# nasa-nccs-hpda/super-resolution-climate

Measured on NVIDIA B200. Metric: rcan_train_tiles_per_s, higher is better.
Workload: dtype bf16

## Files before the change

include/sres_b200.h:

```cpp
#ifndef SRES_B200_H_
#define SRES_B200_H_

#include <stddef.h>
#include <stdint.h>

#ifdef __cplusplus
extern "C" {
#endif

#define SRES_API __attribute__((visibility("default")))

#define SRES_OK 0
#define SRES_ERR_INVALID_ARG 1
#define SRES_ERR_UNSUPPORTED 2
#define SRES_ERR_CUDA 3
#define SRES_ERR_NO_DEVICE 4

#define SRES_NF 64

SRES_API int sres_abi_version(void);
SRES_API const char* sres_last_error(void);
SRES_API int sres_device_sm_count(void);
SRES_API long long sres_launch_count(void);
SRES_API int sres_l2_set_aside(size_t bytes);
SRES_API int sres_l2_persist_window(const void* base, size_t bytes, void* stream);
SRES_API int sres_profile_report(char* buf, size_t nbuf);
SRES_API int64_t sres_ptl_rows(int B, int H, int W);

#define SRES_EPI_RELU 1u
#define SRES_EPI_POOL 2u
#define SRES_EPI_DOT 4u

#define SRES_MAP_IDENT 0
#define SRES_MAP_SHUFFLE 1
#define SRES_MAP_UNSHUFFLE 2

typedef struct sres_conv_args {
  const void* in_bf16;
  const void* wpack_bf16;
  const float* bias;
  const float* resid_f32;
  const float* resid2_f32;
  const void* mask_bf16;
  float* out_f32;
  void* out_bf16;
  float* pool_part;
  float* out_nchw;
  int32_t B, H, W;
  int32_t n_out;
  int32_t c_real;
  uint32_t epi_flags;
  int32_t map_mode;
  int32_t sub_i, sub_j;
  int32_t shuffle_factor;
  int32_t debug_flags;
  void* debug_timeline;
} sres_conv_args;

SRES_API int sres_conv_tile_rows(int H, int W);
SRES_API int sres_conv_mtiles(int B, int H, int W);
SRES_API int sres_conv_supported(int H, int W, int n_out);
SRES_API int sres_conv3x3_igemm(const sres_conv_args* args, void* stream);

SRES_API size_t sres_conv_pair_flag_bytes(int B, int H, int W);
SRES_API int sres_conv_pair_supported(const sres_conv_args* first, const sres_conv_args* second);
SRES_API int sres_conv3x3_pair(const sres_conv_args* first, const sres_conv_args* second, void* flags, void* stream);

typedef struct sres_rcab_chain_args {
  void* xb_bf16;
  void* t1_bf16;
  void* t2_bf16;
  const void* wpack_bf16;
  const float* params;
  const float* x_in_f32;
  float* x_f32;
  float* save_mean;
  float* save_s;
  void* scratch;
  int64_t rcab_stride, save_stride;
  int32_t B, H, W, n_blocks, hidden;
  int32_t xb_first, xb_ring, xb_count;
  int32_t t_first, t_fixed, t_count;
  void* debug_timeline;
} sres_rcab_chain_args;
SRES_API int sres_rcab_chain_supported(int B, int H, int W);
SRES_API size_t sres_rcab_chain_scratch_bytes(int B);
SRES_API int sres_rcab_chain_fwd(const sres_rcab_chain_args* args, void* stream);

SRES_API int sres_pack_conv_weights(const float* w_oihw, void* out_bf16, int mode, int n_rows, int cin,
                           int cout_total, int oc_stride, int oc_offset, void* stream);

SRES_API size_t sres_conv_wgrad_workspace_bytes(void);
#define SRES_WGRAD_MAX_JOBS 8
typedef struct sres_wgrad_job {
  const void* x_bf16;
  const void* dy_bf16;
  float* dw_oihw;
  float* dbias;
  int32_t cout_total, oc_stride, oc_offset, accumulate;
  float scale;
} sres_wgrad_job;
SRES_API int sres_conv3x3_wgrad_batch(const sres_wgrad_job* jobs, int njobs, int B, int H, int W, void* workspace,
                                      size_t workspace_bytes, void* stream);
SRES_API int sres_conv3x3_wgrad(const void* x_bf16, const void* dy_bf16, int B, int H, int W, float* dw_oihw,
                                float* dbias, int cout_total, int oc_stride, int oc_offset, int accumulate,
                                void* workspace, size_t workspace_bytes, void* stream);

SRES_API int sres_conv3x3_small_in(const float* in_nchw, const float* w, const float* bias, int B, int Cs, int H,
                                   int W, int transposed, int unshuffle, float* out_f32, void* out_bf16,
                                   void* stream);
SRES_API int sres_conv3x3_small_out(const void* u_bf16, const float* w, const float* bias, int B, int Cs, int H, int W,
                                    float* out_nchw, void* stream);
SRES_API size_t sres_small_wgrad_workspace_bytes(void);
SRES_API int sres_small_in_wgrad(const float* g1_f32, const float* g2_f32, const float* in_nchw, int B, int Cs,
                                 int H, int W, float* dw, float* db, int accumulate, void* workspace,
                                 size_t workspace_bytes, void* stream);
SRES_API int sres_small_out_wgrad(const float* dout_nchw, const void* u_bf16, int B, int Cs, int H, int W,
                                  float* dw, float* db, int accumulate, void* workspace, size_t workspace_bytes,
                                  void* stream);

SRES_API int sres_ca_blocks_per_image(int B, int H, int W);
SRES_API int sres_ca_pool(const void* t2_bf16, float* pool_sum, int B, int H, int W, void* stream);
SRES_API int sres_ca_apply_fwd(const void* t2_bf16, const float* pool_part, const float* pool_sum, const float* w1,
                               const float* b1, const float* w2, const float* b2, int hidden, const float* x_in,
                               float* x_out, void* xb_out_bf16, float* save_mean, float* save_s, int B, int H, int W,
                               void* stream);
SRES_API int sres_ca_apply_fwd_split(const void* t2_bf16, const float* pool_part, const float* pool_sum, const float* w1,
                                     const float* b1, const float* w2, const float* b2, int hidden, const float* x_in_f32,
                                     const void* xhi_in_bf16, const void* xlo_in_bf16, void* xhi_out_bf16,
                                     void* xlo_out_bf16, float* save_mean, float* save_s, int B, int H, int W,
                                     void* stream);
SRES_API int sres_ca_bwd(const float* grad_f32, const void* t2_bf16, const float* w1, const float* b1,
                         const float* w2, const float* b2, int hidden, const float* save_mean, float* ds_part,
                         void* dt2_bf16, float* save_ds, int B, int H, int W, void* stream);
SRES_API int sres_ca_bwd_apply(const float* grad_f32, const float* tile_part, const float* w1, const float* b1,
                               const float* w2, const float* b2, int hidden, const float* save_mean, void* dt2_bf16,
                               float* save_ds, int B, int H, int W, void* stream);
SRES_API size_t sres_ca_param_grads_scratch_bytes(int nlayers, int B);
SRES_API int sres_ca_param_grads(const float* params_first, float* grads_first, int64_t layer_stride, int nlayers,
                                 const float* save_mean, const float* save_ds, int B, int hidden, int accumulate,
                                 void* scratch, size_t scratch_bytes, void* stream);

SRES_API int sres_bicubic_resize(const float* in, float* out, int planes, int Hi, int Wi, int Ho, int Wo,
                                 double scale_h, double scale_w, void* stream);

SRES_API size_t sres_loss_workspace_bytes(void);
SRES_API int sres_loss_sum(const float* prd, const float* tgt, int planes, int H, int W, int tH, int tW, int kind,
                           double* stat, void* workspace, size_t workspace_bytes, void* stream);
SRES_API int sres_loss_value(const double* stat, double n_total, const double* n_total_dev, int kind, float* loss,
                             void* stream);
SRES_API int sres_loss_grad(const float* prd, const float* tgt, int planes, int H, int W, int tH, int tW, int kind,
                            const float* loss, double n_total, const double* n_total_dev, float gscale,
                            const float* gscale_dev, float* grad,
                            void* stream);

SRES_API int sres_adam_step_flat(float* p, const float* g, float* m, float* v, int64_t n, int64_t step, double lr,
                                 double beta1, double beta2, double eps, double weight_decay, void* stream);

#define SRES_ARCH_RCAN 0
#define SRES_ARCH_EDSR 1
typedef struct sres_rcan_desc {
  int32_t B, H, W;
  int32_t cin, cout;
  int32_t nfeatures;
  int32_t n_groups;
  int32_t n_blocks;
  int32_t reduction;
  int32_t n_up;
  int32_t up_factor[4];
  int32_t arch;
  float res_scale;
} sres_rcan_desc;

SRES_API int64_t sres_rcan_param_count(const sres_rcan_desc* d);
SRES_API int sres_rcan_workspace_bytes(const sres_rcan_desc* d, int training, size_t* bytes);
SRES_API int sres_rcan_pack_weights(const sres_rcan_desc* d, const float* params, void* workspace, int training,
                                    void* stream);
SRES_API int sres_rcan_forward(const sres_rcan_desc* d, const float* params, const float* x_nchw, float* out_nchw,
                               void* workspace, int training, void* stream);
SRES_API int sres_rcan_num_segments(const sres_rcan_desc* d);
SRES_API int sres_rcan_segment_params(const sres_rcan_desc* d, int seg, int64_t* offset, int64_t* count);
SRES_API int sres_async_create(void** ctx);
SRES_API int sres_async_destroy(void* ctx);
SRES_API int sres_rcan_backward(const sres_rcan_desc* d, const float* params, const float* x_nchw,
                                const float* dout_nchw, float* grads, int accumulate, void* workspace, int seg_begin,
                                int seg_end, void* async_ctx, void* stream);

SRES_API int sres_tiles_finite_flags(const float* region, int C, int Y, int X, int y0, int x0, int T, int gy, int gx,
                                     int32_t* flags, void* stream);
SRES_API int sres_tiles_gather(const float* region, int C, int Y, int X, int y0, int x0, int T, int gy, int gx,
                               const int32_t* src_tile, int nslots, float* out, void* stream);
SRES_API int sres_tiles_lnorm(const float* in, int nplanes, int T, int flip_index, float* out, float* mean,
                              float* std_, void* stream);
SRES_API int sres_tiles_stitch(const float* tiles, int C, int ivar, int t, int gy, int gx, const int32_t* cell_to_tile,
                               const float* mean, const float* std_, float* out, void* stream);

SRES_API size_t sres_llc_index_workspace_bytes(int nx);
SRES_API int sres_llc_build_roi_index(const void* template_be, int nx, int y0, int ys, int x0, int xs, void* workspace,
                                      size_t workspace_bytes, int32_t* roi_index, int64_t* n_ocean_dev, void* stream);
SRES_API int sres_llc_gather_roi(const void* data_be, int64_t n_data, const int32_t* roi_index, int64_t npix, float* out,
                                 void* stream);

#ifdef __cplusplus
}
#endif
#endif
```

super-resolution-climate_b200/csrc/ca.cu:

```cuda
#include "internal.h"
#include "ptx.cuh"

namespace sres {

constexpr int kCaThreads = 256;
constexpr int kCaMaxHidden = 64;

struct CaGeom {
  int B, H, W, P, RP;
  int hid;
  int blocks_per_image;
  int tile_rows;
};

__device__ __forceinline__ float warp_sum(float v) {
#pragma unroll
  for (int o = 16; o > 0; o >>= 1) v += __shfl_xor_sync(0xffffffffu, v, o);
  return v;
}
__device__ __forceinline__ void ca_mlp(const float* __restrict__ w1, const float* __restrict__ b1,
                                       const float* __restrict__ w2, const float* __restrict__ b2, int hid,
                                       const float* sm_m, float* sm_h, float* sm_z, float* sm_s) {
  const int lane = threadIdx.x & 31, wrp = threadIdx.x >> 5;
  const float m0 = sm_m[lane], m1 = sm_m[lane + 32];
  for (int j = wrp; j < hid; j += kCaThreads / 32) {
    const float v = warp_sum(fmaf(__ldg(w1 + j * 64 + lane), m0, __ldg(w1 + j * 64 + 32 + lane) * m1));
    if (lane == 0) sm_h[j] = fmaxf(v + __ldg(b1 + j), 0.f);
  }
  __syncthreads();
  for (int c = wrp; c < 64; c += kCaThreads / 32) {
    float v = lane < hid ? __ldg(w2 + c * hid + lane) * sm_h[lane] : 0.f;
    if (lane + 32 < hid) v = fmaf(__ldg(w2 + c * hid + lane + 32), sm_h[lane + 32], v);
    v = warp_sum(v);
    if (lane == 0) {
      const float z = v + __ldg(b2 + c);
      sm_z[c] = z;
      sm_s[c] = 1.f / (1.f + expf(-z));
    }
  }
  __syncthreads();
}

struct CaWeights {
  float* w1;
  float* w2t;
  float* b1;
  float* b2;
};
static size_t ca_weights_bytes(int hid) { return (size_t)(2 * hid * 64 + hid + 64) * sizeof(float); }
__device__ __forceinline__ void ca_stage_weights(CaWeights& S, const float* __restrict__ w1, const float* __restrict__ b1,
                                                 const float* __restrict__ w2, const float* __restrict__ b2, int hid) {
  extern __shared__ float ca_dyn_smem[];
  S.w1 = ca_dyn_smem; S.w2t = S.w1 + hid * 64; S.b1 = S.w2t + hid * 64; S.b2 = S.b1 + hid;
  for (int i = threadIdx.x; i < hid * 64; i += kCaThreads) {
    S.w1[i] = __ldg(w1 + i);
    S.w2t[(i % hid) * 64 + i / hid] = __ldg(w2 + i);
  }
  if (threadIdx.x < hid) S.b1[threadIdx.x] = __ldg(b1 + threadIdx.x);
  if (threadIdx.x < 64) S.b2[threadIdx.x] = __ldg(b2 + threadIdx.x);
}
__device__ __forceinline__ void ca_hidden(const CaWeights& S, int hid, const float* sm_m, float* sm_h) {
  const int lane = threadIdx.x & 31, wrp = threadIdx.x >> 5;
  const float m0 = sm_m[lane], m1 = sm_m[lane + 32];
  for (int j = wrp; j < hid; j += kCaThreads / 32) {
    const float v = warp_sum(fmaf(S.w1[j * 64 + lane], m0, S.w1[j * 64 + 32 + lane] * m1));
    if (lane == 0) sm_h[j] = fmaxf(v + S.b1[j], 0.f);
  }
}
__device__ __forceinline__ float ca_gate(const CaWeights& S, int hid, const float* sm_h, int c) {
  float z = S.b2[c];
  for (int j = 0; j < hid; ++j) z = fmaf(S.w2t[j * 64 + c], sm_h[j], z);
  return 1.f / (1.f + expf(-z));
}

__global__ void __launch_bounds__(kCaThreads)
ca_pool_kernel(CaGeom g, const uint16_t* __restrict__ t2, float* __restrict__ pool_sum) {
  __shared__ float sm[kCaThreads / 8][64 + 1];
  const int b = blockIdx.x, tid = threadIdx.x, cg = tid & 7;
  float a[8] = {0, 0, 0, 0, 0, 0, 0, 0};
  for (int r = tid >> 3; r < g.RP; r += kCaThreads / 8) {
    const uint4 tv = *reinterpret_cast<const uint4*>(t2 + ((size_t)b * g.RP + r) * 64 + cg * 8);
    a[0] += bf16_lo(tv.x); a[1] += bf16_hi(tv.x); a[2] += bf16_lo(tv.y); a[3] += bf16_hi(tv.y);
    a[4] += bf16_lo(tv.z); a[5] += bf16_hi(tv.z); a[6] += bf16_lo(tv.w); a[7] += bf16_hi(tv.w);
  }
#pragma unroll
  for (int j = 0; j < 8; ++j) sm[tid >> 3][cg * 8 + j] = a[j];
  __syncthreads();
  if (tid < 64) {
    float s = 0.f;
    for (int i = 0; i < kCaThreads / 8; ++i) s += sm[i][tid];
    pool_sum[b * 64 + tid] = s;
  }
}


template <bool kSplit>
__global__ void __launch_bounds__(kCaThreads)
ca_apply_fwd_kernel(CaGeom g, const uint16_t* __restrict__ t2, const float* __restrict__ pool_part,
                    const float* __restrict__ pool_sum, const float* __restrict__ w1, const float* __restrict__ b1,
                    const float* __restrict__ w2, const float* __restrict__ b2, const float* x_in, float* x_out,
                    uint16_t* __restrict__ xb_out, float* __restrict__ save_mean, float* __restrict__ save_s,
                    const uint16_t* __restrict__ xhi_in, const uint16_t* xlo_in, uint16_t* xlo_out) {
  __shared__ float sm_red[4][64];
  __shared__ float sm_m[64], sm_h[kCaMaxHidden], sm_s[64];
  CaWeights sw;
  const int b = blockIdx.y, tid = threadIdx.x;
  const int cg = tid & 7;
  ca_stage_weights(sw, w1, b1, w2, b2, g.hid);
  pdl_wait();
  pdl_launch_dependents();
  const int per_blk = (g.RP + g.blocks_per_image - 1) / g.blocks_per_image;
  const int r0 = blockIdx.x * per_blk + (tid >> 3), r1 = min(g.RP, blockIdx.x * per_blk + per_blk);
  if (pool_sum) {
    sm_red[tid >> 6][tid & 63] = (tid < 64) ? pool_sum[b * 64 + tid] : 0.f;
  } else {
    const int c = tid & 63, part = tid >> 6;
    const int t0 = (b * g.RP) / g.tile_rows, t1 = ((b + 1) * g.RP - 1) / g.tile_rows;
    float a = 0.f;
#pragma unroll 8
    for (int t = t0; t <= t1; ++t) {
      const int seg = (t * g.tile_rows >= b * g.RP) ? 0 : 1;
      a += pool_part[(((size_t)t * 2 + seg) * 4 + part) * 64 + c];
    }
    sm_red[part][c] = a;
  }
  __syncthreads();
  if (tid < 64) sm_m[tid] = (sm_red[0][tid] + sm_red[1][tid] + sm_red[2][tid] + sm_red[3][tid]) / float(g.H * g.W);
  __syncthreads();
  ca_hidden(sw, g.hid, sm_m, sm_h);
  __syncthreads();
  if (tid < 64) {
    const float sg = ca_gate(sw, g.hid, sm_h, tid);
    sm_s[tid] = sg;
    if (blockIdx.x == 0) {
      save_mean[b * 64 + tid] = sm_m[tid];
      save_s[b * 64 + tid] = sg;
    }
  }
  __syncthreads();
  if constexpr (kSplit) {
    float s8[8];
#pragma unroll
    for (int j = 0; j < 8; ++j) s8[j] = sm_s[cg * 8 + j];
#pragma unroll 2
    for (int r = r0; r < r1; r += kCaThreads / 8) {
      const size_t q = (size_t)b * g.RP + r;
      const uint4 tv = *reinterpret_cast<const uint4*>(t2 + q * 64 + cg * 8);
      float x[8];
      if (x_in) {
        const float4 xa = *reinterpret_cast<const float4*>(x_in + q * 64 + cg * 8);
        const float4 xb = *reinterpret_cast<const float4*>(x_in + q * 64 + cg * 8 + 4);
        x[0] = xa.x; x[1] = xa.y; x[2] = xa.z; x[3] = xa.w; x[4] = xb.x; x[5] = xb.y; x[6] = xb.z; x[7] = xb.w;
      } else {
        const uint4 hv = *reinterpret_cast<const uint4*>(xhi_in + q * 64 + cg * 8);
        const uint4 lv = *reinterpret_cast<const uint4*>(xlo_in + q * 64 + cg * 8);
        x[0] = bf16_lo(hv.x) + bf16_lo(lv.x); x[1] = bf16_hi(hv.x) + bf16_hi(lv.x);
        x[2] = bf16_lo(hv.y) + bf16_lo(lv.y); x[3] = bf16_hi(hv.y) + bf16_hi(lv.y);
        x[4] = bf16_lo(hv.z) + bf16_lo(lv.z); x[5] = bf16_hi(hv.z) + bf16_hi(lv.z);
        x[6] = bf16_lo(hv.w) + bf16_lo(lv.w); x[7] = bf16_hi(hv.w) + bf16_hi(lv.w);
      }
      float o[8];
      o[0] = fmaf(bf16_lo(tv.x), s8[0], x[0]); o[1] = fmaf(bf16_hi(tv.x), s8[1], x[1]);
      o[2] = fmaf(bf16_lo(tv.y), s8[2], x[2]); o[3] = fmaf(bf16_hi(tv.y), s8[3], x[3]);
      o[4] = fmaf(bf16_lo(tv.z), s8[4], x[4]); o[5] = fmaf(bf16_hi(tv.z), s8[5], x[5]);
      o[6] = fmaf(bf16_lo(tv.w), s8[6], x[6]); o[7] = fmaf(bf16_hi(tv.w), s8[7], x[7]);
      const uint4 h = make_uint4(pack_bf16x2(o[0], o[1]), pack_bf16x2(o[2], o[3]), pack_bf16x2(o[4], o[5]), pack_bf16x2(o[6], o[7]));
      *reinterpret_cast<uint4*>(xb_out + q * 64 + cg * 8) = h;
      *reinterpret_cast<uint4*>(xlo_out + q * 64 + cg * 8) =
          make_uint4(pack_bf16x2(o[0] - bf16_lo(h.x), o[1] - bf16_hi(h.x)), pack_bf16x2(o[2] - bf16_lo(h.y), o[3] - bf16_hi(h.y)),
                     pack_bf16x2(o[4] - bf16_lo(h.z), o[5] - bf16_hi(h.z)), pack_bf16x2(o[6] - bf16_lo(h.w), o[7] - bf16_hi(h.w)));
    }
  } else {
  float s8[8];
#pragma unroll
  for (int j = 0; j < 4; ++j) { s8[j] = sm_s[cg * 4 + j]; s8[4 + j] = sm_s[32 + cg * 4 + j]; }
#pragma unroll 2
  for (int r = r0; r < r1; r += kCaThreads / 8) {
    const size_t q = (size_t)b * g.RP + r;
    const uint2 ta = *reinterpret_cast<const uint2*>(t2 + q * 64 + cg * 4);
    const uint2 tb = *reinterpret_cast<const uint2*>(t2 + q * 64 + 32 + cg * 4);
    const float4 xa = *reinterpret_cast<const float4*>(x_in + q * 64 + cg * 4);
    const float4 xb = *reinterpret_cast<const float4*>(x_in + q * 64 + 32 + cg * 4);
    float o[8];
    o[0] = fmaf(bf16_lo(ta.x), s8[0], xa.x); o[1] = fmaf(bf16_hi(ta.x), s8[1], xa.y);
    o[2] = fmaf(bf16_lo(ta.y), s8[2], xa.z); o[3] = fmaf(bf16_hi(ta.y), s8[3], xa.w);
    o[4] = fmaf(bf16_lo(tb.x), s8[4], xb.x); o[5] = fmaf(bf16_hi(tb.x), s8[5], xb.y);
    o[6] = fmaf(bf16_lo(tb.y), s8[6], xb.z); o[7] = fmaf(bf16_hi(tb.y), s8[7], xb.w);
    *reinterpret_cast<float4*>(x_out + q * 64 + cg * 4) = make_float4(o[0], o[1], o[2], o[3]);
    *reinterpret_cast<float4*>(x_out + q * 64 + 32 + cg * 4) = make_float4(o[4], o[5], o[6], o[7]);
    if (xb_out) {
      *reinterpret_cast<uint2*>(xb_out + q * 64 + cg * 4) = make_uint2(pack_bf16x2(o[0], o[1]), pack_bf16x2(o[2], o[3]));
      *reinterpret_cast<uint2*>(xb_out + q * 64 + 32 + cg * 4) = make_uint2(pack_bf16x2(o[4], o[5]), pack_bf16x2(o[6], o[7]));
    }
  }
  }
}

__global__ void __launch_bounds__(kCaThreads)
ca_bwd_reduce_kernel(CaGeom g, const float* __restrict__ grad, const uint16_t* __restrict__ t2,
                     float* __restrict__ ds_part) {
  __shared__ float sm[kCaThreads / 8][64 + 1];
  pdl_wait();
  pdl_launch_dependents();
  const int b = blockIdx.y, tid = threadIdx.x, cg = tid & 7;
  const int per_blk = (g.RP + g.blocks_per_image - 1) / g.blocks_per_image;
  const int r0 = blockIdx.x * per_blk, r1 = min(g.RP, r0 + per_blk);
  float a[8] = {0, 0, 0, 0, 0, 0, 0, 0};
  for (int r = r0 + (tid >> 3); r < r1; r += kCaThreads / 8) {
    const size_t q = (size_t)b * g.RP + r;
    const uint2 ta = *reinterpret_cast<const uint2*>(t2 + q * 64 + cg * 4);
    const uint2 tb = *reinterpret_cast<const uint2*>(t2 + q * 64 + 32 + cg * 4);
    const float4 ga = *reinterpret_cast<const float4*>(grad + q * 64 + cg * 4);
    const float4 gb = *reinterpret_cast<const float4*>(grad + q * 64 + 32 + cg * 4);
    a[0] = fmaf(ga.x, bf16_lo(ta.x), a[0]); a[1] = fmaf(ga.y, bf16_hi(ta.x), a[1]);
    a[2] = fmaf(ga.z, bf16_lo(ta.y), a[2]); a[3] = fmaf(ga.w, bf16_hi(ta.y), a[3]);
    a[4] = fmaf(gb.x, bf16_lo(tb.x), a[4]); a[5] = fmaf(gb.y, bf16_hi(tb.x), a[5]);
    a[6] = fmaf(gb.z, bf16_lo(tb.y), a[6]); a[7] = fmaf(gb.w, bf16_hi(tb.y), a[7]);
  }
#pragma unroll
  for (int j = 0; j < 4; ++j) { sm[tid >> 3][cg * 4 + j] = a[j]; sm[tid >> 3][32 + cg * 4 + j] = a[4 + j]; }
  __syncthreads();
  if (tid < 64) {
    float s = 0.f;
    for (int i = 0; i < kCaThreads / 8; ++i) s += sm[i][tid];
    ds_part[((size_t)b * g.blocks_per_image + blockIdx.x) * 64 + tid] = s;
  }
}

__global__ void __launch_bounds__(kCaThreads)
ca_bwd_apply_kernel(CaGeom g, const float* __restrict__ grad, const float* __restrict__ ds_part,
                    const float* __restrict__ tile_part, const float* __restrict__ w1, const float* __restrict__ b1, const float* __restrict__ w2,
                    const float* __restrict__ b2, const float* __restrict__ save_mean,
                    uint16_t* __restrict__ dt2, float* __restrict__ save_ds) {
  __shared__ float sm_m[64], sm_h[kCaMaxHidden], sm_s[64], sm_dz[64], sm_dh[kCaMaxHidden], sm_dm[64];
  __shared__ float sm_dsr[4][64];
  CaWeights sw;
  const int b = blockIdx.y, tid = threadIdx.x;
  const int lane = tid & 31, wrp = tid >> 5, cg = tid & 7;
  ca_stage_weights(sw, w1, b1, w2, b2, g.hid);
  pdl_wait();
  pdl_launch_dependents();
  const int per_blk = (g.RP + g.blocks_per_image - 1) / g.blocks_per_image;
  const int r0 = blockIdx.x * per_blk + (tid >> 3), r1 = min(g.RP, blockIdx.x * per_blk + per_blk);
  if (tile_part) {
    const int c = tid & 63, part = tid >> 6;
    const int t0 = (b * g.RP) / g.tile_rows, t1 = ((b + 1) * g.RP - 1) / g.tile_rows;
    float a = 0.f;
#pragma unroll 8
    for (int t = t0; t <= t1; ++t) {
      const int seg = (t * g.tile_rows >= b * g.RP) ? 0 : 1;
      a += tile_part[(((size_t)t * 2 + seg) * 4 + part) * 64 + c];
    }
    sm_dsr[part][c] = a;
  } else if (tid < 64) {
    float a = 0.f;
    for (int i = 0; i < g.blocks_per_image; ++i) a += ds_part[((size_t)b * g.blocks_per_image + i) * 64 + tid];
    sm_dsr[0][tid] = a;
    sm_dsr[1][tid] = sm_dsr[2][tid] = sm_dsr[3][tid] = 0.f;
  }
  if (tid < 64) sm_m[tid] = save_mean[b * 64 + tid];
  __syncthreads();
  ca_hidden(sw, g.hid, sm_m, sm_h);
  __syncthreads();
  if (tid < 64) {
    const float ds = (sm_dsr[0][tid] + sm_dsr[1][tid]) + (sm_dsr[2][tid] + sm_dsr[3][tid]);
    if (blockIdx.x == 0) save_ds[b * 64 + tid] = ds;
    const float sg = ca_gate(sw, g.hid, sm_h, tid);
    sm_s[tid] = sg;
    sm_dz[tid] = ds * sg * (1.f - sg);
  }
  __syncthreads();
  for (int j = wrp; j < g.hid; j += kCaThreads / 32) {
    const float v = warp_sum(fmaf(sw.w2t[j * 64 + lane], sm_dz[lane], sw.w2t[j * 64 + 32 + lane] * sm_dz[lane + 32]));
    if (lane == 0) sm_dh[j] = sm_h[j] > 0.f ? v : 0.f;
  }
  __syncthreads();
  if (tid < 64) {
    float a = 0.f;
    for (int j = 0; j < g.hid; ++j) a = fmaf(sw.w1[j * 64 + tid], sm_dh[j], a);
    sm_dm[tid] = a / float(g.H * g.W);
  }
  __syncthreads();
  float s8[8], m8[8];
#pragma unroll
  for (int j = 0; j < 4; ++j) {
    s8[j] = sm_s[cg * 4 + j]; s8[4 + j] = sm_s[32 + cg * 4 + j];
    m8[j] = sm_dm[cg * 4 + j]; m8[4 + j] = sm_dm[32 + cg * 4 + j];
  }
  int y = r0 / g.P, x = r0 - y * g.P;
#pragma unroll 4
  for (int r = r0; r < r1; r += kCaThreads / 8) {
    const size_t q = (size_t)b * g.RP + r;
    const float4 ga = *reinterpret_cast<const float4*>(grad + q * 64 + cg * 4);
    const float4 gb = *reinterpret_cast<const float4*>(grad + q * 64 + 32 + cg * 4);
    const bool valid = (x != g.W) && (y != g.H);
    uint2 oa, ob;
    oa.x = pack_bf16x2(fmaf(ga.x, s8[0], m8[0]), fmaf(ga.y, s8[1], m8[1]));
    oa.y = pack_bf16x2(fmaf(ga.z, s8[2], m8[2]), fmaf(ga.w, s8[3], m8[3]));
    ob.x = pack_bf16x2(fmaf(gb.x, s8[4], m8[4]), fmaf(gb.y, s8[5], m8[5]));
    ob.y = pack_bf16x2(fmaf(gb.z, s8[6], m8[6]), fmaf(gb.w, s8[7], m8[7]));
    if (!valid) { oa = make_uint2(0, 0); ob = make_uint2(0, 0); }
    *reinterpret_cast<uint2*>(dt2 + q * 64 + cg * 4) = oa;
    *reinterpret_cast<uint2*>(dt2 + q * 64 + 32 + cg * 4) = ob;
    x += kCaThreads / 8;
    while (x >= g.P) { x -= g.P; ++y; }
  }
}

struct CaParamBatch {
  const float* params;
  float* grads;
  long long layer_stride;
  const float* mean;
  const float* ds;
};

__global__ void __launch_bounds__(kCaThreads)
ca_param_prep_kernel(const CaParamBatch batch, int B, int hid, float* __restrict__ scratch) {
  __shared__ float sm_m[64], sm_h[kCaMaxHidden], sm_z[64], sm_s[64], sm_dz[64];
  const int layer = blockIdx.x, b = blockIdx.y, tid = threadIdx.x;
  const long long o = (long long)layer * batch.layer_stride;
  const float* w1 = batch.params + o;
  const float* b1 = w1 + hid * 64;
  const float* w2 = b1 + hid;
  const float* b2 = w2 + 64 * hid;
  if (tid < 64) sm_m[tid] = batch.mean[((size_t)layer * B + b) * 64 + tid];
  __syncthreads();
  ca_mlp(w1, b1, w2, b2, hid, sm_m, sm_h, sm_z, sm_s);
  float* out = scratch + ((size_t)layer * B + b) * (64 + 2 * kCaMaxHidden);
  if (tid < 64) {
    const float s = sm_s[tid];
    const float dz = batch.ds[((size_t)layer * B + b) * 64 + tid] * s * (1.f - s);
    sm_dz[tid] = dz;
    out[tid] = dz;
  }
  __syncthreads();
  if (tid < hid) {
    float a = 0.f;
    for (int c = 0; c < 64; ++c) a = fmaf(w2[c * hid + tid], sm_dz[c], a);
    out[64 + tid] = sm_h[tid];
    out[64 + kCaMaxHidden + tid] = sm_h[tid] > 0.f ? a : 0.f;
  }
}

constexpr int kCaParamChunk = 32;
__global__ void __launch_bounds__(kCaThreads)
ca_param_sum_kernel(const CaParamBatch batch, int B, int hid, const float* __restrict__ scratch, int accumulate) {
  __shared__ float sm[kCaParamChunk][4][64];
  const int layer = blockIdx.x, tid = threadIdx.x;
  const long long o = (long long)layer * batch.layer_stride;
  float* dw1 = batch.grads + o;
  float* db1 = dw1 + hid * 64;
  float* dw2 = db1 + hid;
  float* db2 = dw2 + 64 * hid;
  const int n12 = hid * 64;
  float a1[16], a2[16];
#pragma unroll
  for (int i = 0; i < 16; ++i) a1[i] = a2[i] = 0.f;
  float ab1 = 0.f, ab2 = 0.f;
  for (int b0 = 0; b0 < B; b0 += kCaParamChunk) {
    const int nb = min(kCaParamChunk, B - b0);
    __syncthreads();
    for (int i = tid; i < nb * 256; i += kCaThreads) {
      const int b = i >> 8, k = (i >> 6) & 3, c = i & 63;
      const size_t img = (size_t)layer * B + b0 + b;
      sm[b][k][c] = k < 3 ? scratch[img * (64 + 2 * kCaMaxHidden) + k * 64 + c] : batch.mean[img * 64 + c];
    }
    __syncthreads();
    for (int b = 0; b < nb; ++b) {
      const float* dz = sm[b][0];
      const float* h = sm[b][1];
      const float* dh = sm[b][2];
      const float* m = sm[b][3];
#pragma unroll
      for (int i = 0; i < 16; ++i) {
        const int e = tid + i * kCaThreads;
        if (e < n12) {
          a1[i] = fmaf(dh[e / 64], m[e % 64], a1[i]);
          a2[i] = fmaf(dz[e / hid], h[e % hid], a2[i]);
        }
      }
      if (tid < hid) ab1 += dh[tid];
      if (tid < 64) ab2 += dz[tid];
    }
  }
#pragma unroll
  for (int i = 0; i < 16; ++i) {
    const int e = tid + i * kCaThreads;
    if (e < n12) {
      dw1[e] = accumulate ? dw1[e] + a1[i] : a1[i];
      dw2[e] = accumulate ? dw2[e] + a2[i] : a2[i];
    }
  }
  if (tid < hid) db1[tid] = accumulate ? db1[tid] + ab1 : ab1;
  if (tid < 64) db2[tid] = accumulate ? db2[tid] + ab2 : ab2;
}

static int ca_geom(CaGeom* g, int B, int H, int W, int hid) {
  if (B <= 0 || H <= 0 || W <= 0) return set_error(SRES_ERR_INVALID_ARG, "ca: bad geometry");
  if (hid < 1 || hid > kCaMaxHidden) return set_error(SRES_ERR_UNSUPPORTED, "ca: hidden width must be 1..64");
  g->B = B; g->H = H; g->W = W; g->P = W + 1; g->RP = (H + 1) * (W + 1); g->hid = hid;
  int sms = device_sm_count();
  if (sms <= 0) sms = 148;
  int bpi = (4 * sms + B - 1) / B;
  const int max_bpi = (g->RP + 31) / 32;
  if (bpi > max_bpi) bpi = max_bpi;
  if (bpi < 1) bpi = 1;
  g->blocks_per_image = bpi;
  g->tile_rows = sres_conv_tile_rows(H, W);
  return SRES_OK;
}

}

using namespace sres;

extern "C" int sres_ca_blocks_per_image(int B, int H, int W) {
  CaGeom g;
  if (ca_geom(&g, B, H, W, 1)) return -1;
  return g.blocks_per_image;
}

extern "C" int sres_ca_pool(const void* t2_bf16, float* pool_sum, int B, int H, int W, void* stream) {
  CaGeom g;
  int rc = ca_geom(&g, B, H, W, 1);
  if (rc) return rc;
  if (!t2_bf16 || !pool_sum) return set_error(SRES_ERR_INVALID_ARG, "ca_pool: null pointer");
  ca_pool_kernel<<<B, kCaThreads, 0, (cudaStream_t)stream>>>(g, (const uint16_t*)t2_bf16, pool_sum);
  SRES_CHECK_LAUNCH("ca_pool: launch");
  return SRES_OK;
}

extern "C" int sres_ca_apply_fwd(const void* t2_bf16, const float* pool_part, const float* pool_sum, const float* w1, const float* b1,
                                 const float* w2, const float* b2, int hidden, const float* x_in, float* x_out,
                                 void* xb_out_bf16, float* save_mean, float* save_s, int B, int H, int W,
                                 void* stream) {
  CaGeom g;
  int rc = ca_geom(&g, B, H, W, hidden);
  if (rc) return rc;
  if (!pool_sum && g.RP < 128) return set_error(SRES_ERR_UNSUPPORTED, "ca_apply_fwd: fused pool partials need (H+1)*(W+1) >= 128; pass pool_sum");
  if (!t2_bf16 || (!pool_part && !pool_sum) || !w1 || !b1 || !w2 || !b2 || !x_in || !x_out || !save_mean || !save_s)
    return set_error(SRES_ERR_INVALID_ARG, "ca_apply_fwd: null pointer");
  dim3 grid(g.blocks_per_image, B);
  cudaError_t e = launch_pdl_if(pdl_level() >= 2, ca_apply_fwd_kernel<false>, grid, dim3(kCaThreads), ca_weights_bytes(hidden), (cudaStream_t)stream, g, (const uint16_t*)t2_bf16,
                             pool_part, pool_sum, w1, b1, w2, b2, x_in, x_out, (uint16_t*)xb_out_bf16, save_mean, save_s,
                             (const uint16_t*)nullptr, (const uint16_t*)nullptr, (uint16_t*)nullptr);
  if (e != cudaSuccess) return set_cuda_error(e, "ca_apply_fwd: launch");
  return SRES_OK;
}

extern "C" int sres_ca_apply_fwd_split(const void* t2_bf16, const float* pool_part, const float* pool_sum, const float* w1,
                                       const float* b1, const float* w2, const float* b2, int hidden, const float* x_in_f32,
                                       const void* xhi_in_bf16, const void* xlo_in_bf16, void* xhi_out_bf16,
                                       void* xlo_out_bf16, float* save_mean, float* save_s, int B, int H, int W,
                                       void* stream) {
  CaGeom g;
  int rc = ca_geom(&g, B, H, W, hidden);
  if (rc) return rc;
  if (!pool_sum && g.RP < 128) return set_error(SRES_ERR_UNSUPPORTED, "ca_apply_fwd_split: fused pool partials need (H+1)*(W+1) >= 128; pass pool_sum");
  if (!t2_bf16 || (!pool_part && !pool_sum) || !w1 || !b1 || !w2 || !b2 || !xhi_out_bf16 || !xlo_out_bf16 || !save_mean || !save_s)
    return set_error(SRES_ERR_INVALID_ARG, "ca_apply_fwd_split: null pointer");
  if ((x_in_f32 != nullptr) == (xhi_in_bf16 != nullptr || xlo_in_bf16 != nullptr) || (!x_in_f32 && (!xhi_in_bf16 || !xlo_in_bf16)))
    return set_error(SRES_ERR_INVALID_ARG, "ca_apply_fwd_split: pass either x_in_f32 or both xhi_in_bf16 and xlo_in_bf16");
  if (xhi_in_bf16 == xhi_out_bf16) return set_error(SRES_ERR_INVALID_ARG, "ca_apply_fwd_split: xhi_out must not alias xhi_in");
  dim3 grid(g.blocks_per_image, B);
  cudaError_t e = launch_pdl_if(pdl_level() >= 2, ca_apply_fwd_kernel<true>, grid, dim3(kCaThreads), ca_weights_bytes(hidden), (cudaStream_t)stream, g, (const uint16_t*)t2_bf16,
                             pool_part, pool_sum, w1, b1, w2, b2, x_in_f32, (float*)nullptr, (uint16_t*)xhi_out_bf16, save_mean, save_s,
                             (const uint16_t*)xhi_in_bf16, (const uint16_t*)xlo_in_bf16, (uint16_t*)xlo_out_bf16);
  if (e != cudaSuccess) return set_cuda_error(e, "ca_apply_fwd_split: launch");
  return SRES_OK;
}

extern "C" int sres_ca_bwd(const float* grad_f32, const void* t2_bf16, const float* w1, const float* b1,
                           const float* w2, const float* b2, int hidden, const float* save_mean, float* ds_part,
                           void* dt2_bf16, float* save_ds, int B, int H, int W, void* stream) {
  CaGeom g;
  int rc = ca_geom(&g, B, H, W, hidden);
  if (rc) return rc;
  if (!grad_f32 || !t2_bf16 || !w1 || !b1 || !w2 || !b2 || !save_mean || !ds_part || !dt2_bf16 || !save_ds)
    return set_error(SRES_ERR_INVALID_ARG, "ca_bwd: null pointer");
  dim3 grid(g.blocks_per_image, B);
  cudaError_t e = launch_pdl_if(pdl_level() >= 2, ca_bwd_reduce_kernel, grid, dim3(kCaThreads), 0, (cudaStream_t)stream, g, grad_f32,
                             (const uint16_t*)t2_bf16, ds_part);
  if (e != cudaSuccess) return set_cuda_error(e, "ca_bwd: reduce launch");
  e = launch_pdl_if(pdl_level() >= 2, ca_bwd_apply_kernel, grid, dim3(kCaThreads), ca_weights_bytes(hidden), (cudaStream_t)stream, g, grad_f32, (const float*)ds_part, (const float*)nullptr, w1, b1,
                 w2, b2, save_mean, (uint16_t*)dt2_bf16, save_ds);
  if (e != cudaSuccess) return set_cuda_error(e, "ca_bwd: apply launch");
  return SRES_OK;
}

extern "C" int sres_ca_bwd_apply(const float* grad_f32, const float* tile_part, const float* w1, const float* b1,
                                 const float* w2, const float* b2, int hidden, const float* save_mean, void* dt2_bf16,
                                 float* save_ds, int B, int H, int W, void* stream) {
  CaGeom g;
  int rc = ca_geom(&g, B, H, W, hidden);
  if (rc) return rc;
  if (g.RP < 128) return set_error(SRES_ERR_UNSUPPORTED, "ca_bwd_apply: per-tile partials need (H+1)*(W+1) >= 128");
  if (!grad_f32 || !tile_part || !w1 || !b1 || !w2 || !b2 || !save_mean || !dt2_bf16 || !save_ds)
    return set_error(SRES_ERR_INVALID_ARG, "ca_bwd_apply: null pointer");
  dim3 grid(g.blocks_per_image, B);
  cudaError_t e = launch_pdl_if(pdl_level() >= 2, ca_bwd_apply_kernel, grid, dim3(kCaThreads), ca_weights_bytes(hidden), (cudaStream_t)stream, g, grad_f32,
                                (const float*)nullptr, tile_part, w1, b1, w2, b2, save_mean, (uint16_t*)dt2_bf16, save_ds);
  if (e != cudaSuccess) return set_cuda_error(e, "ca_bwd_apply: launch");
  return SRES_OK;
}

extern "C" size_t sres_ca_param_grads_scratch_bytes(int nlayers, int B) {
  return (size_t)(nlayers > 0 ? nlayers : 0) * (B > 0 ? B : 0) * (64 + 2 * kCaMaxHidden) * sizeof(float);
}

extern "C" int sres_ca_param_grads(const float* params_first, float* grads_first, int64_t layer_stride, int nlayers,
                                   const float* save_mean, const float* save_ds, int B, int hidden, int accumulate,
                                   void* scratch, size_t scratch_bytes, void* stream) {
  if (!params_first || !grads_first || !save_mean || !save_ds || !scratch || nlayers <= 0 || B <= 0)
    return set_error(SRES_ERR_INVALID_ARG, "ca_param_grads: bad argument");
  if (hidden < 1 || hidden > kCaMaxHidden) return set_error(SRES_ERR_UNSUPPORTED, "ca: hidden width must be 1..64");
  if (scratch_bytes < sres_ca_param_grads_scratch_bytes(nlayers, B))
    return set_error(SRES_ERR_INVALID_ARG, "ca_param_grads: scratch too small");
  CaParamBatch batch{params_first, grads_first, (long long)layer_stride, save_mean, save_ds};
  ca_param_prep_kernel<<<dim3(nlayers, B), kCaThreads, 0, (cudaStream_t)stream>>>(batch, B, hidden, (float*)scratch);
  SRES_CHECK_LAUNCH("ca_param_grads: prep launch");
  ca_param_sum_kernel<<<nlayers, kCaThreads, 0, (cudaStream_t)stream>>>(batch, B, hidden, (const float*)scratch, accumulate);
  SRES_CHECK_LAUNCH("ca_param_grads: sum launch");
  return SRES_OK;
}
```

super-resolution-climate_b200/csrc/conv_pair.cu:

```cuda
#include "ptx.cuh"
#include "internal.h"
#include "conv_epi.cuh"

namespace sres {

constexpr int kPStages = 6;
constexpr int kPAcc = 4;
constexpr int kPThreads = 384;
constexpr int kPWBytes = 9 * 64 * 128;

struct PairParams {
  int H, W, P, R, npos, n_tiles;
  int nstage, stage_rows, box_rows;
  int off_s16, off_msk, off_s32, off_tail;
  const float* bias1;
  const float* bias2;
  float* part2;
  unsigned* ready;
  unsigned* consumed;
  long long* timeline;
  int fence_mode;
  int dual_w;
};

constexpr int kPO16 = 1, kPO32 = 2, kPR32 = 4, kPMsk = 8, kPRelu = 16, kPPool = 32, kPDot = 64;

__device__ __forceinline__ unsigned ld_acquire_gpu(const unsigned* p) {
  unsigned v;
  asm volatile("ld.acquire.gpu.global.u32 %0, [%1];" : "=r"(v) : "l"(p) : "memory");
  return v;
}
__device__ __forceinline__ void red_release_gpu_add(unsigned* p, unsigned v) {
  asm volatile("red.release.gpu.global.add.u32 [%0], %1;" ::"l"(p), "r"(v) : "memory");
}
__device__ __forceinline__ void red_relaxed_gpu_add(unsigned* p, unsigned v) {
  asm volatile("red.relaxed.gpu.global.add.u32 [%0], %1;" ::"l"(p), "r"(v) : "memory");
}
__device__ __forceinline__ unsigned ld_relaxed_gpu(const unsigned* p) {
  unsigned v;
  asm volatile("ld.relaxed.gpu.global.u32 %0, [%1];" : "=r"(v) : "l"(p) : "memory");
  return v;
}
__device__ __forceinline__ void fence_proxy_async_mode(int mode) {
  if (mode & 8) return;
  mode &= 3;
  if (mode == 1) asm volatile("fence.proxy.async.global;" ::: "memory");
  else if (mode == 2) asm volatile("fence.proxy.async;" ::: "memory");
}

struct EpiWarp {
  uint8_t* s16; uint8_t* smk; uint8_t* s32;
  uint64_t* bin;
  int n_in;
  int wq, half, lane;
};

template <int FL>
__device__ __forceinline__ void epi_rows(const PairParams& p, EpiWarp& w, const float* s_bias, const CUtensorMap* tmO16,
                                         int tile, uint32_t trow) {
  constexpr bool f_msk = FL & kPMsk, f_relu = FL & kPRelu;
  const int lane = w.lane;
  const int row0 = tile * 128 + w.wq * 32;
  const int q = row0 + lane;
  const int RP = p.R * p.P;
  const int b = q / RP;
  const int rem = q - b * RP;
  const int y = rem / p.P;
  const int x = rem - y * p.P;
  const bool pad = (x == p.W) || (y == p.H) || q >= p.npos;
  uint32_t raw[32];
  tmem_ld32(trow, raw);
  tmem_ld_wait();
  if (f_msk) mbar_wait(w.bin, (w.n_in - 1) & 1, 6);
  const int sw3 = (lane >> 1) & 3;
  uint8_t* r16 = w.s16 + lane * 64;
  const uint8_t* rmk = w.smk + lane * 64;
#pragma unroll
  for (int ch = 0; ch < 2; ++ch) {
    const int c0 = w.half * 32 + ch * 16;
    float v[16];
#pragma unroll
    for (int j = 0; j < 4; ++j) {
      const float4 b4 = *reinterpret_cast<const float4*>(s_bias + c0 + 4 * j);
      v[4 * j + 0] = __uint_as_float(raw[ch * 16 + 4 * j + 0]) + b4.x;
      v[4 * j + 1] = __uint_as_float(raw[ch * 16 + 4 * j + 1]) + b4.y;
      v[4 * j + 2] = __uint_as_float(raw[ch * 16 + 4 * j + 2]) + b4.z;
      v[4 * j + 3] = __uint_as_float(raw[ch * 16 + 4 * j + 3]) + b4.w;
    }
    if (f_relu) {
#pragma unroll
      for (int j = 0; j < 16; ++j) v[j] = fmaxf(v[j], 0.f);
    }
    if (f_msk) {
#pragma unroll
      for (int j = 0; j < 2; ++j) {
        const uint4 mk = *reinterpret_cast<const uint4*>(rmk + (((ch * 2 + j) ^ sw3) << 4));
        const uint32_t w4[4] = {mk.x, mk.y, mk.z, mk.w};
#pragma unroll
        for (int e = 0; e < 4; ++e) {
          if (!(bf16_lo(w4[e]) > 0.f)) v[8 * j + 2 * e] = 0.f;
          if (!(bf16_hi(w4[e]) > 0.f)) v[8 * j + 2 * e + 1] = 0.f;
        }
      }
    }
    if (pad) {
#pragma unroll
      for (int j = 0; j < 16; ++j) v[j] = 0.f;
    }
#pragma unroll
    for (int j = 0; j < 2; ++j)
      *reinterpret_cast<uint4*>(r16 + (((ch * 2 + j) ^ sw3) << 4)) =
          make_uint4(pack_bf16x2(v[8 * j], v[8 * j + 1]), pack_bf16x2(v[8 * j + 2], v[8 * j + 3]),
                     pack_bf16x2(v[8 * j + 4], v[8 * j + 5]), pack_bf16x2(v[8 * j + 6], v[8 * j + 7]));
  }
  (void)tmO16;
}

template <int FL>
__device__ __forceinline__ void epi_frag(const PairParams& p, EpiWarp& w, const float (&bias8)[8], int tile, uint32_t trow) {
  constexpr bool f_o16 = FL & kPO16, f_o32 = FL & kPO32, f_r32 = FL & kPR32, f_msk = FL & kPMsk, f_dot = FL & kPDot;
  constexpr bool use_in = f_msk || f_r32;
  const int lane = w.lane;
  const int fm = lane & 3, frq = lane >> 2;
  const int fcol = ((lane >> 4) & 1) * 16 + ((lane >> 3) & 1) * 8 + 2 * fm + ((lane >> 2) & 1);
  const int row0 = tile * 128 + w.wq * 32;
  const int q = row0 + lane;
  const int RP = p.R * p.P;
  const int b = q / RP;
  const int rem = q - b * RP;
  const int y = rem / p.P;
  const int x = rem - y * p.P;
  const bool pad = (x == p.W) || (y == p.H) || q >= p.npos;
  const int seg = (b != (tile * 128) / RP) ? 1 : 0;
  uint32_t fa[16], fb[16];
  tmem_ld_frag16(trow, fa);
  tmem_ld_frag16(trow + (16u << 16), fb);
  const unsigned padmask = __ballot_sync(0xffffffffu, pad);
  const unsigned seg1 = __ballot_sync(0xffffffffu, seg == 1);
  const bool mixed = seg1 != 0u && seg1 != 0xffffffffu;
  tmem_ld_wait();
  if (use_in) mbar_wait(w.bin, (w.n_in - 1) & 1, 6);
  const int sw3 = (frq >> 1) & 3;
  float cs0[8], cs1[8];
#pragma unroll
  for (int i = 0; i < 8; ++i) cs0[i] = cs1[i] = 0.f;
#pragma unroll
  for (int j = 0; j < 4; ++j) {
    const int r = frq + 8 * j;
    const bool rpad = (padmask >> r) & 1u;
    const bool rs1 = (seg1 >> r) & 1u;
    uint8_t* row32 = w.s32 + r * 128 + (fm & 1) * 8;
    uint8_t* row16 = w.s16 + r * 64 + 4 * fm;
    const uint8_t* rowmk = w.smk + r * 64 + 4 * fm;
#pragma unroll
    for (int k = 0; k < 4; ++k) {
      const uint32_t* src = (j < 2) ? fa : fb;
      float v0 = __uint_as_float(src[4 * k + 2 * (j & 1)]) + bias8[2 * k];
      float v1 = __uint_as_float(src[4 * k + 2 * (j & 1) + 1]) + bias8[2 * k + 1];
      const int o32 = ((2 * k + (fm >> 1)) ^ frq) << 4;
      const int o16 = (k ^ sw3) << 4;
      if (f_r32) {
        const float2 rr = *reinterpret_cast<const float2*>(row32 + o32);
        v0 += rr.x; v1 += rr.y;
      }
      uint32_t mk = 0;
      if (f_msk) mk = *reinterpret_cast<const uint32_t*>(rowmk + o16);
      if (f_msk && !f_dot) {
        if (!(bf16_lo(mk) > 0.f)) v0 = 0.f;
        if (!(bf16_hi(mk) > 0.f)) v1 = 0.f;
      }
      if (rpad) { v0 = 0.f; v1 = 0.f; }
      float c0v = v0, c1v = v1;
      if (f_dot) { c0v = v0 * bf16_lo(mk); c1v = v1 * bf16_hi(mk); }
      if (mixed && rs1) { cs1[2 * k] += c0v; cs1[2 * k + 1] += c1v; }
      else { cs0[2 * k] += c0v; cs0[2 * k + 1] += c1v; }
      if (f_o32) *reinterpret_cast<float2*>(row32 + o32) = make_float2(v0, v1);
      if (f_o16) *reinterpret_cast<uint32_t*>(row16 + o16) = pack_bf16x2(v0, v1);
    }
  }
  const float t0 = frag_colsum(cs0, lane);
  const float t1 = mixed ? frag_colsum(cs1, lane) : 0.f;
  float* dst = p.part2 + ((long long)tile * 2 * 4 + w.wq) * 64 + w.half * 32 + fcol;
  const bool all1 = seg1 == 0xffffffffu;
  dst[0] = all1 ? 0.f : t0;
  dst[4 * 64] = all1 ? t0 : t1;
}

struct SlotUse { int slot; uint32_t use; };
__device__ __forceinline__ SlotUse pair_slot(int mode, int nstage, int phase, int i, int it, int n1) {
  if (mode != 2) return SlotUse{it % nstage, uint32_t(it / nstage)};
  if (phase == 0) {
    if (i >= n1 - 2) {
      const int sl = i - (n1 - 2);
      return SlotUse{sl, uint32_t((n1 - 2 + sl) / 4)};
    }
    const int m = (n1 - 3 - i) & 3;
    return SlotUse{m == 0 ? 3 : m == 1 ? 2 : m == 2 ? 1 : 0, uint32_t(i >> 2)};
  }
  const int m = i & 3;
  const uint32_t b0 = n1 >= 2 ? uint32_t((n1 - 2) / 4 + 1) : 0u, b1 = n1 >= 1 ? uint32_t((n1 - 1) / 4 + 1) : 0u;
  return SlotUse{m == 0 ? 0 : m == 1 ? 1 : m == 2 ? 4 : 5, uint32_t(i >> 2) + (m == 0 ? b0 : m == 1 ? b1 : 0u)};
}

template <int FL1, int FL2>
__global__ void __launch_bounds__(kPThreads, 1)
conv3x3_pair_kernel(const __grid_constant__ CUtensorMap tmA1, const __grid_constant__ CUtensorMap tmW1,
                    const __grid_constant__ CUtensorMap tmO1, const __grid_constant__ CUtensorMap tmM1,
                    const __grid_constant__ CUtensorMap tmA2, const __grid_constant__ CUtensorMap tmW2,
                    const __grid_constant__ CUtensorMap tmO16_2, const __grid_constant__ CUtensorMap tmM2,
                    const __grid_constant__ CUtensorMap tmR32_2, const __grid_constant__ CUtensorMap tmO32_2,
                    const PairParams p) {
  extern __shared__ uint8_t smem_raw[];
  uint8_t* smem = smem_raw + ((1024u - (smem_u32(smem_raw) & 1023u)) & 1023u);
  uint8_t* smem_w = smem;
  uint8_t* smem_w2 = smem + (p.dual_w ? kPWBytes : 0);
  uint8_t* smem_a = smem + kPWBytes * (p.dual_w ? 2 : 1);
  const int stage_bytes = p.stage_rows * 128;
  auto slot_off = [&](int slot) -> int {
    if (slot < 2 || p.dual_w != 2) return slot * stage_bytes;
    return (slot < 4 ? kPWBytes + (slot - 2) * stage_bytes : (slot - 4) * stage_bytes) - 2 * kPWBytes;
  };
  uint8_t* tail = smem + p.off_tail;
  uint64_t* bar_full = reinterpret_cast<uint64_t*>(tail);
  uint64_t* bar_empty = bar_full + kPStages;
  uint64_t* bar_w = bar_empty + kPStages;
  uint64_t* bar_tfull = bar_w + 2;
  uint64_t* bar_tempty = bar_tfull + kPAcc;
  uint64_t* bar_in = bar_tempty + kPAcc;
  uint32_t* tmem_holder = reinterpret_cast<uint32_t*>(bar_in + 8);
  float* s_bias = reinterpret_cast<float*>(tmem_holder + 4);

  const int warp = __shfl_sync(0xffffffffu, threadIdx.x >> 5, 0);
  const int lane = threadIdx.x & 31;
  const int G = gridDim.x;
  const int c1 = blockIdx.x;
  const int c2 = (p.fence_mode & 48) ? p.n_tiles : G - 1 - blockIdx.x;
  const int n1 = c1 < p.n_tiles ? (p.n_tiles - 1 - c1) / G + 1 : 0;
  long long* tl = p.timeline ? p.timeline + (size_t)blockIdx.x * 16 : nullptr;
#define PSTAMP(i)                              \
  do {                                         \
    if (tl && lane == 0) tl[i] = clock64();    \
  } while (0)
  if (tl && threadIdx.x == 0) { tl[0] = clock64(); tl[12] = tl[13] = tl[14] = tl[15] = 0; }

  if (threadIdx.x == 0) {
    tma_prefetch_desc(&tmA1);
    tma_prefetch_desc(&tmW1);
    tma_prefetch_desc(&tmA2);
    tma_prefetch_desc(&tmW2);
    for (int i = 0; i < kPStages; ++i) {
      mbar_init(&bar_full[i], 1);
      mbar_init(&bar_empty[i], 1);
    }
    mbar_init(&bar_w[0], 1);
    mbar_init(&bar_w[1], 1);
    for (int i = 0; i < kPAcc; ++i) {
      mbar_init(&bar_tfull[i], 1);
      mbar_init(&bar_tempty[i], 8);
    }
    for (int i = 0; i < 8; ++i) mbar_init(&bar_in[i], 1);
    mbar_fence_init();
  }
  if (warp == 2) {
    tmem_alloc(tmem_holder, kPAcc * 64);
    tmem_relinquish();
  }
  if (threadIdx.x < 64) s_bias[threadIdx.x] = p.bias1 ? p.bias1[threadIdx.x] : 0.f;
  else if (threadIdx.x < 128) s_bias[threadIdx.x] = p.bias2 ? p.bias2[threadIdx.x - 64] : 0.f;
  tc_fence_before();
  __syncthreads();
  tc_fence_after();
  const uint32_t tmem_base = __shfl_sync(0xffffffffu, *tmem_holder, 0);
  if (warp == 0) PSTAMP(1);
  pdl_launch_dependents();

  if (warp == 0) {
    const bool leader = elect_one();
    if (leader) {
      mbar_expect_tx(&bar_w[0], kPWBytes);
      for (int t = 0; t < 9; ++t) tma_load_2d(smem_w + t * 64 * 128, &tmW1, &bar_w[0], 0, t * 64);
      if (p.dual_w == 1) {
        mbar_expect_tx(&bar_w[1], kPWBytes);
        for (int t = 0; t < 9; ++t) tma_load_2d(smem_w2 + t * 64 * 128, &tmW2, &bar_w[1], 0, t * 64);
      }
    }
    pdl_wait();
    int it = 0;
    for (int tile = c1; tile < p.n_tiles; tile += G, ++it) {
      const SlotUse su = pair_slot(p.dual_w, p.nstage, 0, it, it, n1);
      const int slot = su.slot;
      const uint32_t ph = su.use & 1;
      mbar_wait(&bar_empty[slot], ph ^ 1, 1);
      const int row0 = tile * 128 - (p.P + 1);
      uint8_t* dst = smem_a + slot_off(slot);
      if (leader) {
        mbar_expect_tx(&bar_full[slot], stage_bytes);
        for (int r = 0; r < p.stage_rows; r += p.box_rows) tma_load_2d(dst + r * 128, &tmA1, &bar_full[slot], 0, row0 + r);
      }
      __syncwarp();
    }
    if (p.dual_w == 2) {
      const int ux0 = n1 / 4, ux1 = (n1 + 1) / 4;
      if (ux0 > 0) mbar_wait(&bar_empty[2], uint32_t(ux0 - 1) & 1, 7);
      if (ux1 > 0) mbar_wait(&bar_empty[3], uint32_t(ux1 - 1) & 1, 7);
      PSTAMP(2);
      if (leader) {
        mbar_expect_tx(&bar_w[1], kPWBytes);
        for (int t = 0; t < 9; ++t) tma_load_2d(smem_w2 + t * 64 * 128, &tmW2, &bar_w[1], 0, t * 64);
      }
      __syncwarp();
    }
    if (!p.dual_w) {
      if (n1 > 0) mbar_wait(&bar_empty[(n1 - 1) % p.nstage], ((n1 - 1) / p.nstage) & 1, 7);
      PSTAMP(2);
      if (leader) {
        mbar_expect_tx(&bar_w[1], kPWBytes);
        for (int t = 0; t < 9; ++t) tma_load_2d(smem_w + t * 64 * 128, &tmW2, &bar_w[1], 0, t * 64);
      }
      __syncwarp();
    }
    int prev_t = -1;
    for (int tile = c2, i2 = 0; tile < p.n_tiles; tile += G, ++it, ++i2) {
      const int t = tile - 1 + (lane - 4);
      const bool watch = lane >= 4 && lane < 7 && t >= 0 && t < p.n_tiles;
      unsigned seen = 0;
      long long f0 = 0;
      if (tl) f0 = clock64();
      if (prev_t >= 0) seen = atomicAdd(p.consumed + prev_t, 1u) + 1u;
      if (watch) {
        long long t0 = clock64();
        while (((p.fence_mode & 8) ? ld_relaxed_gpu(p.ready + t) : ld_acquire_gpu(p.ready + t)) < 8u) {
          __nanosleep(32);
          if (clock64() - t0 > 8000000000LL) { atomicExch(&g_sres_dev_error, 0xDEAD0008u); __threadfence_system(); __trap(); }
        }
      }
      if (prev_t >= 0) {
        const unsigned users = (prev_t > 0 ? 1u : 0u) + 1u + (prev_t + 1 < p.n_tiles ? 1u : 0u);
        if (seen == users) { p.ready[prev_t] = 0u; p.consumed[prev_t] = 0u; }
      }
      prev_t = watch ? t : -1;
      if (watch) fence_proxy_async_mode(p.fence_mode);
      __syncwarp();
      if (tl && lane == 4) tl[12] += clock64() - f0;
      const SlotUse su = pair_slot(p.dual_w, p.nstage, 1, i2, it, n1);
      const int slot = su.slot;
      const uint32_t ph = su.use & 1;
      mbar_wait(&bar_empty[slot], ph ^ 1, 1);
      const int row0 = tile * 128 - (p.P + 1);
      uint8_t* dst = smem_a + slot_off(slot);
      if (leader) {
        mbar_expect_tx(&bar_full[slot], stage_bytes);
        for (int r = 0; r < p.stage_rows; r += p.box_rows) tma_load_2d(dst + r * 128, &tmA2, &bar_full[slot], 0, row0 + r);
      }
      __syncwarp();
    }
    if (prev_t >= 0) {
      const unsigned users = (prev_t > 0 ? 1u : 0u) + 1u + (prev_t + 1 < p.n_tiles ? 1u : 0u);
      if (atomicAdd(p.consumed + prev_t, 1u) + 1u == users) { p.ready[prev_t] = 0u; p.consumed[prev_t] = 0u; }
    }
  } else if (warp == 1) {
    const bool leader = elect_one();
    constexpr uint32_t idesc = make_idesc_bf16(128, 64, 0, 0);
    constexpr uint32_t dhi = sdesc_hi_sw128(1024);
    uint32_t w_lo = sdesc_lo(smem_u32(smem_w), 16);
    const uint32_t a_lo0 = sdesc_lo(smem_u32(smem_a), 16);
    const uint32_t row_step = uint32_t(p.P) * 8;
    int it = 0;
#pragma unroll 1
    for (int phase = 0; phase < 2; ++phase) {
      mbar_wait(&bar_w[phase], 0, 2);
      tc_fence_after();
      if (phase == 1) w_lo = sdesc_lo(smem_u32(smem_w2), 16);
      PSTAMP(3 + 3 * phase);
      for (int tile = phase ? c2 : c1, ip = 0; tile < p.n_tiles; tile += G, ++it, ++ip) {
        const SlotUse su = pair_slot(p.dual_w, p.nstage, phase, ip, it, n1);
        const int slot = su.slot;
        const uint32_t ph = su.use & 1;
        const int acc = it % kPAcc;
        const uint32_t aph = (it / kPAcc) & 1;
        long long w0 = 0, w1 = 0;
        if (tl) w0 = clock64();
        mbar_wait(&bar_tempty[acc], aph ^ 1, 3);
        if (tl) w1 = clock64();
        mbar_wait(&bar_full[slot], ph, 4);
        if (tl && lane == 0) { tl[14] += w1 - w0; tl[15] += clock64() - w1; }
        tc_fence_after();
        const uint32_t a_tile = p.dual_w == 2 ? sdesc_lo(smem_u32(smem_a) + slot_off(slot), 16) : a_lo0 + uint32_t(slot * stage_bytes) / 16;
        const uint32_t d_tmem = tmem_base + uint32_t(acc * 64);
        if (leader) {
#pragma unroll
          for (int t = 0; t < 9; ++t) {
            const uint32_t a_tap = a_tile + uint32_t(t / 3) * row_step + uint32_t(t % 3) * 8;
            const uint32_t b_tap = w_lo + uint32_t(t * 64 * 8);
#pragma unroll
            for (int k = 0; k < 4; ++k) {
              if (t == 0 && k == 0) umma_bf16_lohi<false>(d_tmem, a_tap, dhi, b_tap, dhi, idesc);
              else umma_bf16_lohi<true>(d_tmem, a_tap + k * 2, dhi, b_tap + k * 2, dhi, idesc);
            }
          }
          umma_commit(&bar_empty[slot]);
          umma_commit(&bar_tfull[acc]);
        }
        __syncwarp();
      }
      PSTAMP(4 + 3 * phase);
    }
  } else if (warp >= 4) {
    EpiWarp w;
    const int ew = warp - 4;
    w.wq = warp & 3; w.half = ew >> 2; w.lane = lane; w.n_in = 0;
    w.s16 = smem + p.off_s16 + ew * 2048;
    w.smk = smem + p.off_msk + ew * 2048;
    w.s32 = smem + p.off_s32 + ew * 4096;
    w.bin = &bar_in[ew];
    constexpr bool in1 = FL1 & kPMsk;
    constexpr bool in2 = (FL2 & kPMsk) || (FL2 & kPR32);
    pdl_wait();
    int it = 0;
    constexpr int kLag = 5;
    int pend[kLag];
#pragma unroll
    for (int i = 0; i < kLag; ++i) pend[i] = -1;
    for (int tile = c1; tile < p.n_tiles; tile += G, ++it) {
      const int acc = it % kPAcc;
      const uint32_t aph = (it / kPAcc) & 1;
      const int row0 = tile * 128 + w.wq * 32;
      if (lane == 0) {
        bulk_wait_read<0>();
        if (pend[0] >= 0 && !(p.fence_mode & 16)) {
          if (!(p.fence_mode & 128)) bulk_wait_all<kLag - 1>();
          fence_proxy_async_mode(p.fence_mode);
          if (p.fence_mode & (64 | 8)) red_relaxed_gpu_add(p.ready + pend[0], 1u);
          else red_release_gpu_add(p.ready + pend[0], 1u);
        }
        if (in1) {
          mbar_expect_tx(w.bin, 2048u);
          tma_load_2d(w.smk, &tmM1, w.bin, w.half * 32, row0);
        }
      }
      if (in1) ++w.n_in;
      __syncwarp();
      mbar_wait(&bar_tfull[acc], aph, 5);
      tc_fence_after();
      const uint32_t trow = tmem_base + (uint32_t(w.wq * 32) << 16) + uint32_t(acc * 64 + w.half * 32);
      epi_rows<FL1>(p, w, s_bias, &tmO1, tile, trow);
      tc_fence_before();
      __syncwarp();
      if (lane == 0) mbar_arrive(&bar_tempty[acc]);
      fence_proxy_async_smem();
      __syncwarp();
      if (lane == 0) {
        tma_store_2d(&tmO1, w.s16, w.half * 32, row0);
        bulk_commit();
      }
#pragma unroll
      for (int i = 0; i + 1 < kLag; ++i) pend[i] = pend[i + 1];
      pend[kLag - 1] = tile;
    }
    if (lane == 0 && !(p.fence_mode & 48)) {
      bulk_wait_all<0>();
      fence_proxy_async_mode(p.fence_mode);
#pragma unroll
      for (int i = 0; i < kLag; ++i)
        if (pend[i] >= 0) {
          if (p.fence_mode & 8) red_relaxed_gpu_add(p.ready + pend[i], 1u);
          else red_release_gpu_add(p.ready + pend[i], 1u);
        }
    }
    __syncwarp();
    if (warp == 4) PSTAMP(5);
    const int fm = lane & 3;
    float bias8[8];
#pragma unroll
    for (int i = 0; i < 8; ++i) bias8[i] = s_bias[64 + w.half * 32 + 8 * (i >> 1) + 2 * fm + (i & 1)];
    for (int tile = c2; tile < p.n_tiles; tile += G, ++it) {
      const int acc = it % kPAcc;
      const uint32_t aph = (it / kPAcc) & 1;
      const int row0 = tile * 128 + w.wq * 32;
      if (lane == 0) {
        bulk_wait_read<0>();
        if (in2) {
          mbar_expect_tx(w.bin, ((FL2 & kPMsk) ? 2048u : 0u) + ((FL2 & kPR32) ? 4096u : 0u));
          if (FL2 & kPMsk) tma_load_2d(w.smk, &tmM2, w.bin, w.half * 32, row0);
          if (FL2 & kPR32) tma_load_2d(w.s32, &tmR32_2, w.bin, w.half * 32, row0);
        }
      }
      if (in2) ++w.n_in;
      __syncwarp();
      mbar_wait(&bar_tfull[acc], aph, 5);
      tc_fence_after();
      const uint32_t trow = tmem_base + (uint32_t(w.wq * 32) << 16) + uint32_t(acc * 64 + w.half * 32);
      epi_frag<FL2>(p, w, bias8, tile, trow);
      tc_fence_before();
      __syncwarp();
      if (lane == 0) mbar_arrive(&bar_tempty[acc]);
      fence_proxy_async_smem();
      __syncwarp();
      if (lane == 0) {
        if (FL2 & kPO16) tma_store_2d(&tmO16_2, w.s16, w.half * 32, row0);
        if (FL2 & kPO32) tma_store_2d(&tmO32_2, w.s32, w.half * 32, row0);
        bulk_commit();
      }
    }
    if (lane == 0) bulk_wait_all<0>();
    if (warp == 4) PSTAMP(8);
  }

  tc_fence_before();
  __syncthreads();
  if (tl && threadIdx.x == 0) tl[9] = clock64();
  if (warp == 2) tmem_dealloc(tmem_base, kPAcc * 64);
#undef PSTAMP
}

static bool pair_plan(int W, bool fwd, PairParams* p, size_t* smem_bytes) {
  const int smem_max = 232448;
  const int slab = fwd ? 16384 : (16384 + 16384 + 32768);
  const int rows = 128 + 2 * (W + 2);
  const int box = (rows + 7) / 8 * 8 <= 256 ? (rows + 7) / 8 * 8 : 64;
  const int stage_rows = (rows + box - 1) / box * box;
  static const int dual_env = [] { const char* e = getenv("SRES_PAIR_DUALW"); return e ? atoi(e) : 2; }();
  int dual = 0;
  int ns = (smem_max - 1024 - kPWBytes - 1024 - slab) / (stage_rows * 128);
  if (dual_env) {
    const int ns2 = (smem_max - 1024 - 2 * kPWBytes - 1024 - slab) / (stage_rows * 128);
    if (ns2 >= 2) {
      dual = (dual_env >= 2 && 2 * stage_rows * 128 <= kPWBytes) ? 2 : 1;
      ns = dual == 2 ? 2 : ns2;
    }
  }
  if (ns > kPStages) ns = kPStages;
  if (ns < 2) return false;
  if (p) {
    p->box_rows = box; p->stage_rows = stage_rows; p->nstage = ns; p->dual_w = dual;
    int off = kPWBytes * (dual ? 2 : 1) + ns * stage_rows * 128;
    p->off_s16 = off; off += 16384;
    p->off_msk = off; off += fwd ? 0 : 16384;
    p->off_s32 = off; off += fwd ? 0 : 32768;
    p->off_tail = off; off += 1024;
    *smem_bytes = (size_t)off + 1024;
  }
  return true;
}

static bool conv_pair_fuse_enabled() {
  static const int on = [] {
    const char* e = getenv("SRES_CONV_FUSE");
    return e ? atoi(e) : 1;
  }();
  return on != 0;
}

}

using namespace sres;

extern "C" size_t sres_conv_pair_flag_bytes(int B, int H, int W) {
  const long long npos = (long long)B * (H + 1) * (W + 1);
  return (size_t)((npos + 127) / 128) * 2 * sizeof(unsigned);
}

extern "C" int sres_conv_pair_supported(const sres_conv_args* a1, const sres_conv_args* a2) {
  if (!conv_pair_fuse_enabled() || !a1 || !a2) return 0;
  if (a1->B != a2->B || a1->H != a2->H || a1->W != a2->W || a1->W + 2 > 128) return 0;
  if (a1->n_out != 64 || a2->n_out != 64 || a1->map_mode != SRES_MAP_IDENT || a2->map_mode != SRES_MAP_IDENT) return 0;
  if (a1->out_bf16 == nullptr || a2->in_bf16 != a1->out_bf16) return 0;
  if (a1->out_f32 || a1->resid_f32 || a1->resid2_f32 || a1->out_nchw || a2->resid2_f32 || a2->out_nchw) return 0;
  if (a1->debug_flags || a2->debug_flags) return 0;
  const long long npos = (long long)a1->B * (a1->H + 1) * (a1->W + 1);
  if ((a1->H + 1) * (a1->W + 1) < 128 || npos > 0x7fffff00LL) return 0;
  const bool fwd = (a1->epi_flags == SRES_EPI_RELU) && !a1->mask_bf16 && a2->epi_flags == SRES_EPI_POOL && a2->out_bf16 &&
                   !a2->out_f32 && !a2->resid_f32 && !a2->mask_bf16 && a2->pool_part;
  const bool bwd = a1->epi_flags == 0 && a1->mask_bf16 && a2->epi_flags == SRES_EPI_DOT && a2->mask_bf16 && a2->out_f32 &&
                   a2->resid_f32 && !a2->out_bf16 && a2->pool_part;
  return ((fwd || bwd) && pair_plan(a1->W, fwd, nullptr, nullptr)) ? 1 : 0;
}

extern "C" int sres_conv3x3_pair(const sres_conv_args* a1, const sres_conv_args* a2, void* flags, void* stream_) {
  if (!sres_conv_pair_supported(a1, a2) || !flags) return set_error(SRES_ERR_UNSUPPORTED, "conv pair: flavours / geometry not fusable");
  cudaStream_t stream = (cudaStream_t)stream_;
  const bool fwd = a1->epi_flags == SRES_EPI_RELU;
  PairParams p{};
  p.H = a1->H; p.W = a1->W; p.P = a1->W + 1; p.R = a1->H + 1;
  p.npos = (int)((long long)a1->B * p.R * p.P);
  p.n_tiles = (p.npos + 127) / 128;
  p.bias1 = a1->bias; p.bias2 = a2->bias; p.part2 = a2->pool_part;
  p.ready = (unsigned*)flags; p.consumed = p.ready + p.n_tiles;
  p.timeline = (long long*)a1->debug_timeline;
  {
    static const int fm = [] { const char* e = getenv("SRES_PAIR_FENCE"); return e ? atoi(e) : 8; }();
    p.fence_mode = fm;
  }
  const int smem_max = 232448;
  size_t smem = 0;
  if (!pair_plan(a1->W, fwd, &p, &smem)) return set_error(SRES_ERR_UNSUPPORTED, "conv pair: no room for the halo ring");

  CUtensorMap tmA1, tmW1, tmO1, tmM1, tmA2, tmW2, tmO16_2, tmM2, tmR32_2, tmO32_2;
  int rc;
  if ((rc = make_tmap_rows64(&tmA1, a1->in_bf16, (uint64_t)p.npos, p.box_rows))) return rc;
  if ((rc = make_tmap_rows64(&tmW1, a1->wpack_bf16, 9 * 64, 64))) return rc;
  if ((rc = make_tmap_rows64_half(&tmO1, a1->out_bf16, (uint64_t)p.npos, 32))) return rc;
  tmM1 = tmO1;
  if (a1->mask_bf16 && (rc = make_tmap_rows64_half(&tmM1, a1->mask_bf16, (uint64_t)p.npos, 32))) return rc;
  if ((rc = make_tmap_rows64(&tmA2, a2->in_bf16, (uint64_t)p.npos, p.box_rows))) return rc;
  if ((rc = make_tmap_rows64(&tmW2, a2->wpack_bf16, 9 * 64, 64))) return rc;
  tmO16_2 = tmO1; tmM2 = tmO1; tmR32_2 = tmO1; tmO32_2 = tmO1;
  if (a2->out_bf16 && (rc = make_tmap_rows64_half(&tmO16_2, a2->out_bf16, (uint64_t)p.npos, 32))) return rc;
  if (a2->mask_bf16 && (rc = make_tmap_rows64_half(&tmM2, a2->mask_bf16, (uint64_t)p.npos, 32))) return rc;
  if (a2->resid_f32 && (rc = make_tmap_rows64_f32(&tmR32_2, a2->resid_f32, (uint64_t)p.npos, 32))) return rc;
  if (a2->out_f32 && (rc = make_tmap_rows64_f32(&tmO32_2, a2->out_f32, (uint64_t)p.npos, 32))) return rc;

  const int sms = device_sm_count();
  if (sms <= 0) return set_error(SRES_ERR_NO_DEVICE, "conv pair: no CUDA device");
  const int grid = p.n_tiles < sms ? p.n_tiles : sms;
  int dev = 0;
  cudaGetDevice(&dev);
  cudaLaunchConfig_t cfg{};
  cfg.gridDim = dim3(grid); cfg.blockDim = dim3(kPThreads); cfg.dynamicSmemBytes = smem; cfg.stream = stream;
  cudaLaunchAttribute at[1];
  at[0].id = cudaLaunchAttributeProgrammaticStreamSerialization;
  at[0].val.programmaticStreamSerializationAllowed = 1;
  cfg.attrs = at;
  cfg.numAttrs = pdl_enabled() ? 1 : 0;
  cudaError_t e;
  if (fwd) {
    auto k = conv3x3_pair_kernel<kPRelu | kPO16, kPPool | kPO16>;
    static thread_local int attr_dev = -1;
    if (attr_dev != dev) {
      if ((e = cudaFuncSetAttribute(k, cudaFuncAttributeMaxDynamicSharedMemorySize, smem_max)) != cudaSuccess) return set_cuda_error(e, "conv pair: smem attribute");
      attr_dev = dev;
    }
    count_launch();
    e = cudaLaunchKernelEx(&cfg, k, tmA1, tmW1, tmO1, tmM1, tmA2, tmW2, tmO16_2, tmM2, tmR32_2, tmO32_2, p);
  } else {
    auto k = conv3x3_pair_kernel<kPMsk | kPO16, kPR32 | kPO32 | kPMsk | kPDot>;
    static thread_local int attr_dev = -1;
    if (attr_dev != dev) {
      if ((e = cudaFuncSetAttribute(k, cudaFuncAttributeMaxDynamicSharedMemorySize, smem_max)) != cudaSuccess) return set_cuda_error(e, "conv pair: smem attribute");
      attr_dev = dev;
    }
    count_launch();
    e = cudaLaunchKernelEx(&cfg, k, tmA1, tmW1, tmO1, tmM1, tmA2, tmW2, tmO16_2, tmM2, tmR32_2, tmO32_2, p);
  }
  if (e != cudaSuccess) return set_cuda_error(e, "conv pair: launch");
  e = cudaGetLastError();
  if (e != cudaSuccess) return set_cuda_error(e, "conv pair: launch");
  return SRES_OK;
}
```

super-resolution-climate_b200/csrc/rcan_net.cu:

```cuda
#include <stdio.h>
#include <stdlib.h>
#include <string.h>
#include <map>
#include <mutex>
#include <string>
#include <vector>
#include "internal.h"
#include "ptx.cuh"

namespace sres {

#ifndef SRES_RCAB_CHAIN_DEFAULT
#define SRES_RCAB_CHAIN_DEFAULT 0
#endif
constexpr int kConvW = 64 * 64 * 9;
constexpr int kRing = 8;
static int ring_len() {
  static const int v = [] {
    const char* e = getenv("SRES_RING");
    int n = e ? atoi(e) : 5;
    return n < 3 ? 3 : (n > kRing ? kRing : n);
  }();
  return v;
}
static bool trunk_split() {
  static const bool v = [] { const char* e = getenv("SRES_TRUNK_SPLIT"); return e && atoi(e) != 0; }();
  return v;
}
static bool rcab_chain_enabled() {
  const char* e = getenv("SRES_RCAB_CHAIN");
  return e ? atoi(e) != 0 : SRES_RCAB_CHAIN_DEFAULT != 0;
}
static bool join_per_segment() {
  static const bool v = [] { const char* e = getenv("SRES_JOIN_PER_SEG"); return e && atoi(e) != 0; }();
  return v;
}
static int wgrad_batch_jobs() {
  static const int v = [] {
    const char* e = getenv("SRES_WGRAD_BATCH");
    int n = e ? atoi(e) : 8;
    return n < 1 ? 1 : (n > SRES_WGRAD_MAX_JOBS ? SRES_WGRAD_MAX_JOBS : n);
  }();
  return v;
}

struct ProfRec { const char* cat; cudaEvent_t a, b; };
static std::vector<ProfRec>* t_prof = nullptr;
static std::mutex g_prof_mu;
static bool prof_on() {
  static const bool v = [] { const char* e = getenv("SRES_PROFILE"); return e && atoi(e) > 0; }();
  return v;
}
struct ProfScope {
  cudaStream_t st; ProfRec r; bool on;
  ProfScope(const char* cat, void* stream) : st((cudaStream_t)stream), on(prof_on()) {
    if (!on) return;
    cudaStreamCaptureStatus cs = cudaStreamCaptureStatusNone;
    cudaStreamIsCapturing(st, &cs);
    if (cs != cudaStreamCaptureStatusNone) { on = false; return; }
    r.cat = cat;
    cudaEventCreate(&r.a); cudaEventCreate(&r.b);
    cudaEventRecord(r.a, st);
  }
  ~ProfScope() {
    if (!on) return;
    cudaEventRecord(r.b, st);
    std::lock_guard<std::mutex> lk(g_prof_mu);
    if (!t_prof) t_prof = new std::vector<ProfRec>();
    t_prof->push_back(r);
  }
};
#define PROF(cat) ProfScope prof_scope__(cat, st)

#define RC0(x)           \
  do {                   \
    int rc__ = (x);      \
    if (rc__) return rc__; \
  } while (0)

struct Net {
  sres_rcan_desc d;
  bool edsr;
  float rs;
  int per;
  int hid;
  long long head_w, head_b, body0, rcab_sz, group_sz, bt_w, bt_b, up_w[4], up_b[4], tail_w, tail_b, n_params;
  int n_body_convs;
  int lvH[5], lvW[5];
  long long lvRows[5];
  size_t o_wp_fwd, o_wp_dg, o_wp_up_fwd[4], o_wp_up_dg[4], o_wp_tail, o_bias_up[4], o_bias_tail;
  size_t o_xb, o_t1, o_t2, o_mean, o_s, o_ds, o_resb, o_u[4];
  size_t o_hf, o_gf[2], o_xf, o_pool_part, o_pool_sum;
  size_t o_sbias;
  size_t o_pair_flags;
  size_t o_ga, o_gb32, o_gb16, o_dt2[kRing], o_dt1[kRing], o_ds_part, o_wg_ws, o_sw_ws, o_ca_scr, o_du16[4], o_du32[4], o_dres32, o_dres16;
  size_t total;
  int n_xb, n_t;
  long long cidx(int g, int r, int which) const { return (long long)g * per + 2 * r + which; }
  long long cidx_gt(int g) const { return (long long)g * per + 2 * d.n_blocks; }
  long long cidx_bt() const { return (long long)d.n_groups * per; }
  long long off_rcab(int g, int r) const { return body0 + g * group_sz + r * rcab_sz; }
  long long off_gt(int g) const { return body0 + g * group_sz + d.n_blocks * rcab_sz; }
};

static size_t align_up(size_t v, size_t a = 1024) { return (v + a - 1) / a * a; }

static int build_net(Net* n, const sres_rcan_desc* d, int training) {
  if (!d) return set_error(SRES_ERR_INVALID_ARG, "rcan: null description");
  if (d->B <= 0 || d->H <= 0 || d->W <= 0) return set_error(SRES_ERR_INVALID_ARG, "rcan: bad tile geometry");
  if (d->nfeatures != 64) return set_error(SRES_ERR_UNSUPPORTED, "rcan: kernels are specialised for nfeatures == 64");
  if (d->cin < 1 || d->cin > 4 || d->cout < 1 || d->cout > 4)
    return set_error(SRES_ERR_UNSUPPORTED, "rcan: 1..4 image channels supported");
  if (d->n_groups < 1 || d->n_blocks < 1) return set_error(SRES_ERR_INVALID_ARG, "rcan: need >= 1 group and block");
  if (d->arch != SRES_ARCH_RCAN && d->arch != SRES_ARCH_EDSR) return set_error(SRES_ERR_INVALID_ARG, "rcan: unknown arch");
  const bool edsr = d->arch == SRES_ARCH_EDSR;
  if (!edsr && (d->reduction < 1 || 64 % d->reduction)) return set_error(SRES_ERR_INVALID_ARG, "rcan: reduction must divide 64");
  if (edsr && d->n_groups != 1) return set_error(SRES_ERR_INVALID_ARG, "edsr: n_groups must be 1 (n_blocks = number of ResBlocks)");
  if (edsr && !(d->res_scale > 0.f)) return set_error(SRES_ERR_INVALID_ARG, "edsr: res_scale must be positive");
  if (d->n_up < 0 || d->n_up > 4) return set_error(SRES_ERR_UNSUPPORTED, "rcan: at most 4 upsampler stages");
  memset(n, 0, sizeof(*n));
  n->d = *d;
  n->edsr = edsr;
  n->rs = edsr ? d->res_scale : 1.f;
  n->hid = edsr ? 0 : 64 / d->reduction;
  n->per = 2 * d->n_blocks + (edsr ? 0 : 1);
  const int G = d->n_groups, R = d->n_blocks, hid = n->hid;
  long long o = 0;
  n->head_w = o; o += 64LL * d->cin * 9;
  n->head_b = o; o += 64;
  n->body0 = o;
  n->rcab_sz = 2LL * (kConvW + 64) + (edsr ? 0 : (hid * 64 + hid) + (64 * hid + 64));
  n->group_sz = R * n->rcab_sz + (edsr ? 0 : kConvW + 64);
  o += G * n->group_sz;
  n->bt_w = o; o += kConvW;
  n->bt_b = o; o += 64;
  n->lvH[0] = d->H; n->lvW[0] = d->W;
  for (int i = 0; i < d->n_up; ++i) {
    const int f = d->up_factor[i];
    if (f != 2 && f != 3) return set_error(SRES_ERR_UNSUPPORTED, "rcan: upsampler stage factor must be 2 or 3");
    n->up_w[i] = o; o += (long long)f * f * kConvW;
    n->up_b[i] = o; o += f * f * 64;
    n->lvH[i + 1] = n->lvH[i] * f; n->lvW[i + 1] = n->lvW[i] * f;
  }
  n->tail_w = o; o += (long long)d->cout * 64 * 9;
  n->tail_b = o; o += d->cout;
  n->n_params = o;
  n->n_body_convs = G * n->per + 1;
  for (int i = 0; i <= d->n_up; ++i) {
    n->lvRows[i] = (long long)d->B * (n->lvH[i] + 1) * (n->lvW[i] + 1);
    if (n->lvRows[i] > 0x7fffff00LL) return set_error(SRES_ERR_UNSUPPORTED, "rcan: batch too large");
  }
  const size_t r0 = (size_t)n->lvRows[0];
  const size_t bf = r0 * 128, f32 = r0 * 256;
  size_t w = 0;
  auto take = [&](size_t bytes) { size_t at = w; w = align_up(w + bytes); return at; };
  n->o_wp_fwd = take((size_t)n->n_body_convs * kConvW * 2);
  n->o_wp_dg = take((size_t)n->n_body_convs * kConvW * 2);
  for (int i = 0; i < d->n_up; ++i) {
    const int f2 = d->up_factor[i] * d->up_factor[i];
    n->o_wp_up_fwd[i] = take((size_t)f2 * kConvW * 2);
    n->o_wp_up_dg[i] = take((size_t)f2 * kConvW * 2);
    n->o_bias_up[i] = take((size_t)f2 * 64 * 4);
  }
  n->o_wp_tail = take(9 * 16 * 64 * 2);
  n->o_bias_tail = take(16 * 4);
  n->n_xb = training ? G * (R + 1) + 1 : 2;
  n->n_t = training ? G * R : 1;
  n->o_xb = take((size_t)n->n_xb * bf);
  n->o_t1 = take((size_t)n->n_t * bf);
  if (edsr) {
    n->o_sbias = take((size_t)R * 64 * 4);
  } else {
    n->o_t2 = take((size_t)n->n_t * bf);
    n->o_mean = take((size_t)n->n_t * d->B * 64 * 4);
    n->o_s = take((size_t)n->n_t * d->B * 64 * 4);
  }
  n->o_resb = take(bf);
  for (int i = 0; i < d->n_up; ++i) n->o_u[i] = take((size_t)n->lvRows[i + 1] * 128);
  n->o_hf = take(f32);
  n->o_gf[0] = take(f32);
  n->o_gf[1] = take(f32);
  n->o_xf = take(f32);
  n->o_pool_part = take((size_t)sres_conv_mtiles(d->B, d->H, d->W) * 2 * 4 * 64 * 4);
  n->o_pool_sum = take((size_t)d->B * 64 * 4);
  n->o_pair_flags = take(2 * sres_conv_pair_flag_bytes(d->B, d->H, d->W));
  if (training) {
    n->o_ga = take(f32);
    n->o_gb16 = take(bf);
    for (int k = 0; k < ring_len(); ++k) { n->o_dt2[k] = take(bf); n->o_dt1[k] = take(bf); }
    if (!edsr) {
      n->o_ds = take((size_t)n->n_t * d->B * 64 * 4);
      n->o_gb32 = take(f32);
      const int bpi = sres_ca_blocks_per_image(d->B, d->H, d->W);
      n->o_ds_part = take((size_t)d->B * (bpi > 0 ? bpi : 1) * 64 * 4);
      n->o_ca_scr = take(sres_ca_param_grads_scratch_bytes(R, d->B));
    }
    n->o_wg_ws = take(sres_conv_wgrad_workspace_bytes());
    n->o_sw_ws = take(sres_small_wgrad_workspace_bytes());
    for (int i = 0; i < d->n_up; ++i) {
      const int f2 = d->up_factor[i] * d->up_factor[i];
      n->o_du16[i] = take((size_t)f2 * n->lvRows[i] * 128);
      if (i < d->n_up - 1) n->o_du32[i] = take((size_t)f2 * n->lvRows[i] * 256);
    }
    n->o_dres32 = take(f32);
    n->o_dres16 = take(bf);
  }
  n->total = w;
  return SRES_OK;
}

struct PackBody {
  const float* params;
  long long body0, rcab_sz, group_sz, bt_w;
  int G, R, per;
  float scale2;
  float* sbias;
  uint16_t* fwd;
  uint16_t* dg;
};
__global__ void pack_body_kernel(PackBody pb) {
  const int conv = blockIdx.y;
  const int per = pb.per;
  long long off;
  float sc = 1.f;
  if (conv == pb.G * per) off = pb.bt_w;
  else {
    const int g = conv / per, k = conv % per;
    off = pb.body0 + g * pb.group_sz + (k < 2 * pb.R ? (k / 2) * pb.rcab_sz + (k & 1) * (kConvW + 64) : pb.R * pb.rcab_sz);
    if (k < 2 * pb.R && (k & 1)) {
      sc = pb.scale2;
      if (pb.sbias && blockIdx.x == 0 && threadIdx.x < 64)
        pb.sbias[(size_t)(g * pb.R + k / 2) * 64 + threadIdx.x] = sc * pb.params[off + kConvW + threadIdx.x];
    }
  }
  const float* w = pb.params + off;
  for (int idx = blockIdx.x * blockDim.x + threadIdx.x; idx < kConvW; idx += gridDim.x * blockDim.x) {
    const int k = idx & 63, n = (idx >> 6) & 63, t = idx >> 12;
    const int ky = t / 3, kx = t % 3;
    const float vf = sc * w[((n * 64 + k) * 3 + ky) * 3 + kx];
    const float vd = sc * w[((k * 64 + n) * 3 + (2 - ky)) * 3 + (2 - kx)];
    pb.fwd[(size_t)conv * kConvW + idx] = (uint16_t)(pack_bf16x2(vf, 0.f) & 0xFFFF);
    pb.dg[(size_t)conv * kConvW + idx] = (uint16_t)(pack_bf16x2(vd, 0.f) & 0xFFFF);
  }
}
__global__ void gather_bias_kernel(const float* __restrict__ b, float* __restrict__ out, int n_out, int stride, int offset,
                                   int n_src) {
  const int i = blockIdx.x * blockDim.x + threadIdx.x;
  if (i < n_out) {
    const int s = i * stride + offset;
    out[i] = s < n_src ? b[s] : 0.f;
  }
}

static int pack_all(const Net& n, const float* params, uint8_t* ws, cudaStream_t st) {
  PackBody pb{params, n.body0, n.rcab_sz, n.group_sz, n.bt_w, n.d.n_groups, n.d.n_blocks, n.per, n.rs,
              n.edsr ? (float*)(ws + n.o_sbias) : nullptr, (uint16_t*)(ws + n.o_wp_fwd), (uint16_t*)(ws + n.o_wp_dg)};
  pack_body_kernel<<<dim3(8, n.n_body_convs), 256, 0, st>>>(pb);
  SRES_CHECK_LAUNCH("rcan: pack launch");
  for (int i = 0; i < n.d.n_up; ++i) {
    const int f = n.d.up_factor[i], f2 = f * f;
    for (int sub = 0; sub < f2; ++sub) {
      int rc = sres_pack_conv_weights(params + n.up_w[i], ws + n.o_wp_up_fwd[i] + (size_t)sub * kConvW * 2, 0, 64, 64,
                                      f2 * 64, f2, sub, st);
      if (rc) return rc;
      rc = sres_pack_conv_weights(params + n.up_w[i], ws + n.o_wp_up_dg[i] + (size_t)sub * kConvW * 2, 1, 64, 64,
                                  f2 * 64, f2, sub, st);
      if (rc) return rc;
      gather_bias_kernel<<<1, 64, 0, st>>>(params + n.up_b[i], (float*)(ws + n.o_bias_up[i]) + sub * 64, 64, f2, sub,
                                           f2 * 64);
      SRES_CHECK_LAUNCH("rcan: bias gather launch");
    }
  }
  int rc = sres_pack_conv_weights(params + n.tail_w, ws + n.o_wp_tail, 0, 16, 64, n.d.cout, 1, 0, st);
  if (rc) return rc;
  gather_bias_kernel<<<1, 64, 0, st>>>(params + n.tail_b, (float*)(ws + n.o_bias_tail), 16, 1, 0, n.d.cout);
  SRES_CHECK_LAUNCH("rcan: bias gather launch");
  return SRES_OK;
}

static sres_conv_args conv64_args(const void* in, const void* wp, const float* bias, int B, int H, int W, float* out_f32,
                                  void* out_bf16, unsigned flags = 0, float* pool = nullptr, const float* resid = nullptr,
                                  const float* resid2 = nullptr, const void* mask = nullptr, int map = SRES_MAP_IDENT,
                                  int si = 0, int sj = 0, int sf = 2) {
  sres_conv_args a;
  memset(&a, 0, sizeof(a));
  a.in_bf16 = in; a.wpack_bf16 = wp; a.bias = bias; a.resid_f32 = resid; a.resid2_f32 = resid2; a.mask_bf16 = mask;
  a.out_f32 = out_f32; a.out_bf16 = out_bf16; a.pool_part = pool;
  a.B = B; a.H = H; a.W = W; a.n_out = 64; a.epi_flags = flags; a.map_mode = map; a.sub_i = si; a.sub_j = sj;
  a.shuffle_factor = sf;
  return a;
}

static int conv64(const void* in, const void* wp, const float* bias, int B, int H, int W, void* st, float* out_f32,
                  void* out_bf16, unsigned flags = 0, float* pool = nullptr, const float* resid = nullptr,
                  const float* resid2 = nullptr, const void* mask = nullptr, int map = SRES_MAP_IDENT, int si = 0,
                  int sj = 0, int sf = 2) {
  PROF(map != SRES_MAP_IDENT ? "conv shuffle/unshuffle" : (flags & SRES_EPI_DOT) ? "conv dgrad +fp32 rmw +ds-dot" : mask ? "conv dgrad+relu-mask" : (resid && out_f32) ? "conv +fp32 addend (rmw)"
       : (flags & SRES_EPI_POOL) ? "conv fwd +pool" : (flags & SRES_EPI_RELU) ? "conv fwd +relu" : "conv other");
  const sres_conv_args a = conv64_args(in, wp, bias, B, H, W, out_f32, out_bf16, flags, pool, resid, resid2, mask, map, si, sj, sf);
  return sres_conv3x3_igemm(&a, st);
}

static int conv64_pair(const sres_conv_args& a1, const sres_conv_args& a2, void* flags, void* st, const char* cat) {
  if (sres_conv_pair_supported(&a1, &a2)) {
    PROF(cat);
    return sres_conv3x3_pair(&a1, &a2, flags, st);
  }
  { PROF((a1.epi_flags & SRES_EPI_RELU) ? "conv fwd +relu" : "conv dgrad+relu-mask"); RC0(sres_conv3x3_igemm(&a1, st)); }
  PROF((a2.epi_flags & SRES_EPI_DOT) ? "conv dgrad +fp32 rmw +ds-dot" : "conv fwd +pool");
  return sres_conv3x3_igemm(&a2, st);
}

#define RC(x)            \
  do {                   \
    int rc__ = (x);      \
    if (rc__) return rc__; \
  } while (0)

static int forward(const Net& n, const float* P, const float* x, float* out, uint8_t* ws, int training, void* st) {
  const sres_rcan_desc& d = n.d;
  const int B = d.B, H = d.H, W = d.W, G = d.n_groups, R = d.n_blocks;
  const size_t bf = (size_t)n.lvRows[0] * 128;
  const bool fused_pool = (H + 1) * (W + 1) >= 128;
  auto XB = [&](int i) { return ws + n.o_xb + (size_t)(training ? i : (i & 1)) * bf; };
  auto T1 = [&](int i) { return ws + n.o_t1 + (size_t)(training ? i : 0) * bf; };
  auto T2 = [&](int i) { return ws + n.o_t2 + (size_t)(training ? i : 0) * bf; };
  auto WF = [&](long long c) { return ws + n.o_wp_fwd + (size_t)c * kConvW * 2; };
  float* hf = (float*)(ws + n.o_hf);
  float* xf = (float*)(ws + n.o_xf);
  float* pool_part = (float*)(ws + n.o_pool_part);
  float* pool_sum = (float*)(ws + n.o_pool_sum);
  int xbi = 0;
  const bool l2hint = l2_hint_enabled();
  const bool split = trunk_split() && !n.edsr;
  if (l2hint) RC(sres_l2_persist_window(xf, (size_t)n.lvRows[0] * (split ? 128 : 256), st));
  { PROF("head conv"); RC(sres_conv3x3_small_in(x, P + n.head_w, P + n.head_b, B, d.cin, H, W, 0, 0, hf, XB(0), st)); }
  const float* gin = hf;
  if (n.edsr) {
    for (int r = 0; r < R; ++r) {
      const float* pr = P + n.off_rcab(0, r);
      RC(conv64(XB(xbi), WF(n.cidx(0, r, 0)), pr + kConvW, B, H, W, st, nullptr, T1(r), SRES_EPI_RELU));
      RC(conv64(T1(r), WF(n.cidx(0, r, 1)), (const float*)(ws + n.o_sbias) + (size_t)r * 64, B, H, W, st, xf, XB(xbi + 1), 0,
                nullptr, r == 0 ? hf : xf));
      ++xbi;
    }
  }
  const bool chain = !n.edsr && rcab_chain_enabled() && fused_pool && sres_rcab_chain_supported(B, H, W);
  for (int g = 0; g < (n.edsr ? 0 : G); ++g) {
    float* gout = (float*)(ws + n.o_gf[g & 1]);
    if (chain) {
      PROF("rcab chain fwd (R blocks)");
      sres_rcab_chain_args ca;
      memset(&ca, 0, sizeof(ca));
      ca.xb_bf16 = ws + n.o_xb; ca.t1_bf16 = ws + n.o_t1; ca.t2_bf16 = ws + n.o_t2;
      ca.wpack_bf16 = WF(n.cidx(g, 0, 0));
      ca.params = P + n.off_rcab(g, 0);
      ca.x_in_f32 = gin; ca.x_f32 = xf;
      ca.save_mean = (float*)(ws + n.o_mean) + (size_t)(training ? g * R : 0) * B * 64;
      ca.save_s = (float*)(ws + n.o_s) + (size_t)(training ? g * R : 0) * B * 64;
      ca.scratch = pool_part;
      ca.rcab_stride = n.rcab_sz; ca.save_stride = training ? (long long)B * 64 : 0;
      ca.B = B; ca.H = H; ca.W = W; ca.n_blocks = R; ca.hidden = n.hid;
      ca.xb_first = xbi; ca.xb_ring = training ? 0 : 2; ca.xb_count = n.n_xb;
      ca.t_first = training ? g * R : 0; ca.t_fixed = training ? 0 : 1; ca.t_count = n.n_t;
      RC(sres_rcab_chain_fwd(&ca, st));
      xbi += R;
    }
    for (int r = 0; r < (chain ? 0 : R); ++r) {
      const int ti = g * R + r;
      const float* pr = P + n.off_rcab(g, r);
      const float* c1b = pr + kConvW;
      const float* c2b = pr + 2 * kConvW + 64;
      const float* w1 = pr + 2 * (kConvW + 64);
      const float* b1 = w1 + n.hid * 64;
      const float* w2 = b1 + n.hid;
      const float* b2 = w2 + 64 * n.hid;
      RC(conv64_pair(conv64_args(XB(xbi), WF(n.cidx(g, r, 0)), c1b, B, H, W, nullptr, T1(ti), SRES_EPI_RELU),
                     conv64_args(T1(ti), WF(n.cidx(g, r, 1)), c2b, B, H, W, nullptr, T2(ti), fused_pool ? SRES_EPI_POOL : 0,
                                 fused_pool ? pool_part : nullptr),
                     ws + n.o_pair_flags + (size_t)(ti & 1) * sres_conv_pair_flag_bytes(B, H, W), st, "conv pair fwd (conv1 -> conv2 +pool)"));
      if (!fused_pool) RC(sres_ca_pool(T2(ti), pool_sum, B, H, W, st));
      float* mean = (float*)(ws + n.o_mean) + (size_t)(training ? ti : 0) * B * 64;
      float* sv = (float*)(ws + n.o_s) + (size_t)(training ? ti : 0) * B * 64;
      { PROF("ca_apply_fwd");
      if (split)
        RC(sres_ca_apply_fwd_split(T2(ti), fused_pool ? pool_part : nullptr, fused_pool ? nullptr : pool_sum, w1, b1, w2, b2,
                                   n.hid, r == 0 ? gin : nullptr, r == 0 ? nullptr : XB(xbi), r == 0 ? nullptr : (const void*)xf,
                                   XB(xbi + 1), xf, mean, sv, B, H, W, st));
      else
        RC(sres_ca_apply_fwd(T2(ti), fused_pool ? pool_part : nullptr, fused_pool ? nullptr : pool_sum, w1, b1, w2, b2,
                             n.hid, r == 0 ? gin : xf, xf, XB(xbi + 1), mean, sv, B, H, W, st)); }
      ++xbi;
    }
    const float* pg = P + n.off_gt(g);
    RC(conv64(XB(xbi), WF(n.cidx_gt(g)), pg + kConvW, B, H, W, st, gout, XB(xbi + 1), 0, nullptr, gin));
    ++xbi;
    gin = gout;
  }
  if (l2hint) RC(sres_l2_persist_window(nullptr, 0, st));
  void* resb = ws + n.o_resb;
  RC(conv64(XB(xbi), WF(n.cidx_bt()), P + n.bt_b, B, H, W, st, nullptr, resb, 0, nullptr, hf));
  const void* cur = resb;
  for (int i = 0; i < d.n_up; ++i) {
    const int f = d.up_factor[i];
    for (int sub = 0; sub < f * f; ++sub)
      RC(conv64(cur, ws + n.o_wp_up_fwd[i] + (size_t)sub * kConvW * 2, (const float*)(ws + n.o_bias_up[i]) + sub * 64, B,
                n.lvH[i], n.lvW[i], st, nullptr, ws + n.o_u[i], 0, nullptr, nullptr, nullptr, nullptr, SRES_MAP_SHUFFLE,
                sub / f, sub % f, f));
    cur = ws + n.o_u[i];
  }
  sres_conv_args a;
  memset(&a, 0, sizeof(a));
  a.in_bf16 = cur; a.wpack_bf16 = ws + n.o_wp_tail; a.bias = (const float*)(ws + n.o_bias_tail);
  a.out_nchw = out; a.c_real = d.cout; a.n_out = 16;
  a.B = B; a.H = n.lvH[d.n_up]; a.W = n.lvW[d.n_up];
  if (sres_conv_supported(a.H, a.W, 16)) {
    PROF("tail conv (N=16)");
    RC(sres_conv3x3_igemm(&a, st));
  } else {
    PROF("tail conv (CUDA cores)");
    RC(sres_conv3x3_small_out(cur, P + n.tail_w, P + n.tail_b, B, d.cout, a.H, a.W, out, st));
  }
  return SRES_OK;
}

struct AsyncCtx {
  static constexpr int kEvents = 8;
  cudaStream_t side = nullptr;
  cudaEvent_t fork[kEvents], done[kEvents];
  const void* bufs[kEvents][SRES_WGRAD_MAX_JOBS];
  bool live[kEvents];
  int next = 0;
};

struct WgQueue {
  sres_wgrad_job jobs[SRES_WGRAD_MAX_JOBS];
  int n = 0, B = 0, H = 0, W = 0;
  const Net* net = nullptr;
  uint8_t* ws = nullptr;
  void* st = nullptr;
  AsyncCtx* ax = nullptr;
  int wait_slot(int i) {
    if (ax && ax->live[i]) {
      cudaError_t e = cudaStreamWaitEvent((cudaStream_t)st, ax->done[i], 0);
      if (e != cudaSuccess) return set_cuda_error(e, "backward: join side stream");
      ax->live[i] = false;
    }
    return SRES_OK;
  }
  int join_all() {
    if (ax)
      for (int i = 0; i < AsyncCtx::kEvents; ++i) RC(wait_slot(i));
    return SRES_OK;
  }
  int flush() {
    if (n == 0) return SRES_OK;
    PROF("wgrad batch (+reduce)");
    int rc;
    if (ax) {
      const int i = ax->next;
      ax->next = (i + 1) % AsyncCtx::kEvents;
      RC(wait_slot(i));
      cudaError_t e = cudaEventRecord(ax->fork[i], (cudaStream_t)st);
      if (e == cudaSuccess) e = cudaStreamWaitEvent(ax->side, ax->fork[i], 0);
      if (e != cudaSuccess) return set_cuda_error(e, "backward: fork side stream");
      rc = sres_conv3x3_wgrad_batch(jobs, n, B, H, W, ws + net->o_wg_ws, sres_conv_wgrad_workspace_bytes(), ax->side);
      if (rc) return rc;
      e = cudaEventRecord(ax->done[i], ax->side);
      if (e != cudaSuccess) return set_cuda_error(e, "backward: side event");
      for (int k = 0; k < SRES_WGRAD_MAX_JOBS; ++k) ax->bufs[i][k] = k < n ? jobs[k].dy_bf16 : nullptr;
      ax->live[i] = true;
    } else {
      rc = sres_conv3x3_wgrad_batch(jobs, n, B, H, W, ws + net->o_wg_ws, sres_conv_wgrad_workspace_bytes(), st);
    }
    n = 0;
    return rc;
  }
  template <class F>
  int run_side(F fn) {
    if (!ax || join_per_segment()) return fn(st);
    const int i = ax->next;
    ax->next = (i + 1) % AsyncCtx::kEvents;
    RC(wait_slot(i));
    cudaError_t e = cudaEventRecord(ax->fork[i], (cudaStream_t)st);
    if (e == cudaSuccess) e = cudaStreamWaitEvent(ax->side, ax->fork[i], 0);
    if (e != cudaSuccess) return set_cuda_error(e, "backward: fork side stream");
    RC(fn((void*)ax->side));
    e = cudaEventRecord(ax->done[i], ax->side);
    if (e != cudaSuccess) return set_cuda_error(e, "backward: side event");
    for (int k = 0; k < SRES_WGRAD_MAX_JOBS; ++k) ax->bufs[i][k] = nullptr;
    ax->live[i] = true;
    return SRES_OK;
  }
  int push(const void* x, const void* dy, int B_, int H_, int W_, float* dw, float* db, int cout_total, int stride,
           int offset, int acc, float scale = 1.f) {
    if (n && (B_ != B || H_ != H || W_ != W)) RC(flush());
    B = B_; H = H_; W = W_;
    sres_wgrad_job& j = jobs[n++];
    j.x_bf16 = x; j.dy_bf16 = dy; j.dw_oihw = dw; j.dbias = db;
    j.cout_total = cout_total; j.oc_stride = stride; j.oc_offset = offset; j.accumulate = acc;
    j.scale = scale;
    if (n == wgrad_batch_jobs()) RC(flush());
    return SRES_OK;
  }
  int before_write(const void* buf) {
    for (int i = 0; i < n; ++i)
      if (jobs[i].dy_bf16 == buf) { RC(flush()); break; }
    if (ax)
      for (int i = 0; i < AsyncCtx::kEvents; ++i)
        if (ax->live[i])
          for (int k = 0; k < SRES_WGRAD_MAX_JOBS; ++k)
            if (ax->bufs[i][k] == buf) { RC(wait_slot(i)); break; }
    return SRES_OK;
  }
};

static int backward(const Net& n, const float* P, const float* x, const float* dout, float* Gr, int accumulate,
                    uint8_t* ws, int seg_begin, int seg_end, AsyncCtx* ax, void* st) {
  const sres_rcan_desc& d = n.d;
  const int B = d.B, H = d.H, W = d.W, G = d.n_groups, R = d.n_blocks, L = d.n_up;
  const size_t bf = (size_t)n.lvRows[0] * 128;
  auto XB = [&](int i) { return ws + n.o_xb + (size_t)i * bf; };
  auto T1 = [&](int i) { return ws + n.o_t1 + (size_t)i * bf; };
  auto T2 = [&](int i) { return ws + n.o_t2 + (size_t)i * bf; };
  auto WD = [&](long long c) { return ws + n.o_wp_dg + (size_t)c * kConvW * 2; };
  float* ga = (float*)(ws + n.o_ga);
  float* gb32 = (float*)(ws + n.o_gb32);
  void* gb16 = ws + n.o_gb16;
  WgQueue wq;
  wq.net = &n; wq.ws = ws; wq.st = st; wq.ax = ax;
  if (ax) for (int i = 0; i < AsyncCtx::kEvents; ++i) ax->live[i] = false;
  float* dres32 = (float*)(ws + n.o_dres32);
  void* dres16 = ws + n.o_dres16;
  const int xb_last = n.edsr ? R : G * (R + 1);
  const bool fused_dot = (H + 1) * (W + 1) >= 128;

  for (int seg = seg_begin; seg < seg_end; ++seg) {
    if (seg == 0) {
      const int Hh = n.lvH[L], Wh = n.lvW[L];
      const void* u_last = L > 0 ? (const void*)(ws + n.o_u[L - 1]) : (const void*)(ws + n.o_resb);
      { PROF("tail wgrad");
      RC(sres_small_out_wgrad(dout, u_last, B, d.cout, Hh, Wh, Gr + n.tail_w, Gr + n.tail_b, accumulate, ws + n.o_sw_ws,
                              sres_small_wgrad_workspace_bytes(), st)); }
      { PROF("tail dgrad");
      if (L == 0) {
        RC(sres_conv3x3_small_in(dout, P + n.tail_w, nullptr, B, d.cout, Hh, Wh, 1, 0, dres32, dres16, st));
      } else {
        RC(sres_conv3x3_small_in(dout, P + n.tail_w, nullptr, B, d.cout, Hh, Wh, 1, d.up_factor[L - 1], nullptr,
                                 ws + n.o_du16[L - 1], st));
      } }
      for (int i = L - 1; i >= 0; --i) {
        const int f = d.up_factor[i], f2 = f * f;
        const void* cur_in = i > 0 ? (const void*)(ws + n.o_u[i - 1]) : (const void*)(ws + n.o_resb);
        const size_t sub_bytes = (size_t)n.lvRows[i] * 128;
        float* acc32 = i > 0 ? (float*)(ws + n.o_du32[i - 1]) : dres32;
        void* acc16 = i > 0 ? (void*)(ws + n.o_du16[i - 1]) : dres16;
        const int map = i > 0 ? SRES_MAP_UNSHUFFLE : SRES_MAP_IDENT;
        const int sf = i > 0 ? d.up_factor[i - 1] : 2;
        for (int sub = 0; sub < f2; ++sub) {
          const void* dy = ws + n.o_du16[i] + sub * sub_bytes;
          RC(wq.push(cur_in, dy, B, n.lvH[i], n.lvW[i], Gr + n.up_w[i], Gr + n.up_b[i], f2 * 64, f2, sub, accumulate));
          RC(conv64(dy, ws + n.o_wp_up_dg[i] + (size_t)sub * kConvW * 2, nullptr, B, n.lvH[i], n.lvW[i], st, acc32,
                    sub == f2 - 1 ? acc16 : nullptr, 0, nullptr, sub > 0 ? acc32 : nullptr, nullptr, nullptr, map, 0, 0,
                    sf));
        }
      }
      RC(wq.push(XB(xb_last), dres16, B, H, W, Gr + n.bt_w, Gr + n.bt_b, 64, 1, 0, accumulate));
      RC(wq.before_write(gb16));
      RC(conv64(dres16, WD(n.cidx_bt()), nullptr, B, H, W, st, ga, gb16));
      RC(wq.flush());
      if (join_per_segment()) RC(wq.join_all());
    } else if (seg <= G && n.edsr) {
      const bool l2hint = l2_hint_enabled();
      if (l2hint) RC(sres_l2_persist_window(ga, (size_t)n.lvRows[0] * 256, st));
      for (int r = R - 1; r >= 0; --r) {
        float* gr = Gr + n.off_rcab(0, r);
        const void* g16 = r == R - 1 ? gb16 : (const void*)(ws + n.o_dt2[r % ring_len()]);
        void* dt1 = ws + n.o_dt1[r % ring_len()];
        RC(wq.push(T1(r), g16, B, H, W, gr + kConvW + 64, gr + 2 * kConvW + 64, 64, 1, 0, accumulate, n.rs));
        RC(wq.before_write(dt1));
        RC(conv64(g16, WD(n.cidx(0, r, 1)), nullptr, B, H, W, st, nullptr, dt1, 0, nullptr, nullptr, nullptr, T1(r)));
        RC(wq.push(XB(r), dt1, B, H, W, gr, gr + kConvW, 64, 1, 0, accumulate));
        void* nxt = r > 0 ? (void*)(ws + n.o_dt2[(r - 1) % ring_len()]) : nullptr;
        if (nxt) RC(wq.before_write(nxt));
        RC(conv64(dt1, WD(n.cidx(0, r, 0)), nullptr, B, H, W, st, ga, nxt, 0, nullptr, ga));
      }
      RC(wq.flush());
      if (l2hint) RC(sres_l2_persist_window(nullptr, 0, st));
    } else if (seg <= G) {
      const int g = G - seg;
      const int xb0 = g * (R + 1);
      const bool l2hint = l2_hint_enabled();
      if (l2hint) RC(sres_l2_persist_window(gb32, (size_t)n.lvRows[0] * 256, st));
      float* Gg = Gr + n.off_gt(g);
      RC(wq.push(XB(xb0 + R), gb16, B, H, W, Gg, Gg + kConvW, 64, 1, 0, accumulate));
      float* dot_part = (float*)(ws + n.o_pool_part);
      RC(conv64(gb16, WD(n.cidx_gt(g)), nullptr, B, H, W, st, gb32, nullptr, fused_dot ? SRES_EPI_DOT : 0,
                fused_dot ? dot_part : nullptr, nullptr, nullptr, fused_dot ? T2(g * R + R - 1) : nullptr));
      for (int r = R - 1; r >= 0; --r) {
        const int ti = g * R + r;
        const float* pr = P + n.off_rcab(g, r);
        float* gr = Gr + n.off_rcab(g, r);
        const float* w1 = pr + 2 * (kConvW + 64);
        const float* b1 = w1 + n.hid * 64;
        const float* w2 = b1 + n.hid;
        const float* b2 = w2 + 64 * n.hid;
        const float* mean = (const float*)(ws + n.o_mean) + (size_t)ti * B * 64;
        float* dsv = (float*)(ws + n.o_ds) + (size_t)ti * B * 64;
        void* dt2 = ws + n.o_dt2[ti % ring_len()];
        void* dt1 = ws + n.o_dt1[ti % ring_len()];
        RC(wq.before_write(dt2));
        { PROF("ca_bwd");
        if (fused_dot) RC(sres_ca_bwd_apply(gb32, dot_part, w1, b1, w2, b2, n.hid, mean, dt2, dsv, B, H, W, st));
        else RC(sres_ca_bwd(gb32, T2(ti), w1, b1, w2, b2, n.hid, mean, (float*)(ws + n.o_ds_part), dt2, dsv, B, H, W, st)); }
        RC(wq.push(T1(ti), dt2, B, H, W, gr + kConvW + 64, gr + 2 * kConvW + 64, 64, 1, 0, accumulate));
        RC(wq.before_write(dt1));
        if (r > 0) {
          RC(conv64_pair(conv64_args(dt2, WD(n.cidx(g, r, 1)), nullptr, B, H, W, nullptr, dt1, 0, nullptr, nullptr, nullptr, T1(ti)),
                         conv64_args(dt1, WD(n.cidx(g, r, 0)), nullptr, B, H, W, gb32, nullptr, fused_dot ? SRES_EPI_DOT : 0,
                                     fused_dot ? dot_part : nullptr, gb32, nullptr, fused_dot ? T2(ti - 1) : nullptr),
                         ws + n.o_pair_flags + (size_t)(ti & 1) * sres_conv_pair_flag_bytes(B, H, W), st,
                         "conv pair bwd (dgrad2 -> dgrad1 +rmw +dot)"));
          RC(wq.push(XB(xb0 + r), dt1, B, H, W, gr, gr + kConvW, 64, 1, 0, accumulate));
        } else {
          RC(conv64(dt2, WD(n.cidx(g, r, 1)), nullptr, B, H, W, st, nullptr, dt1, 0, nullptr, nullptr, nullptr, T1(ti)));
          RC(wq.push(XB(xb0 + r), dt1, B, H, W, gr, gr + kConvW, 64, 1, 0, accumulate));
          RC(wq.before_write(gb16));
          RC(conv64(dt1, WD(n.cidx(g, r, 0)), nullptr, B, H, W, st, ga, gb16, 0, nullptr, gb32, ga));
        }
      }
      RC(wq.flush());
      if (l2hint) RC(sres_l2_persist_window(nullptr, 0, st));
      const long long first = n.off_rcab(g, 0) + 2 * (kConvW + 64);
      PROF("ca_param_grads");
      if (join_per_segment()) RC(wq.join_all());
      RC(wq.run_side([&](void* s) {
        return sres_ca_param_grads(P + first, Gr + first, n.rcab_sz, R, (const float*)(ws + n.o_mean) + (size_t)g * R * B * 64,
                                   (const float*)(ws + n.o_ds) + (size_t)g * R * B * 64, B, n.hid, accumulate,
                                   ws + n.o_ca_scr, sres_ca_param_grads_scratch_bytes(R, B), s);
      }));
    } else if (seg == G + 1) {
      PROF("head wgrad");
      RC(sres_small_in_wgrad(ga, dres32, x, B, d.cin, H, W, Gr + n.head_w, Gr + n.head_b, accumulate, ws + n.o_sw_ws,
                             sres_small_wgrad_workspace_bytes(), st));
    }
  }
  RC(wq.join_all());
  return SRES_OK;
}

}

using namespace sres;

extern "C" int64_t sres_rcan_param_count(const sres_rcan_desc* d) {
  Net n;
  if (build_net(&n, d, 0)) return -1;
  return n.n_params;
}

extern "C" int sres_rcan_workspace_bytes(const sres_rcan_desc* d, int training, size_t* bytes) {
  Net n;
  int rc = build_net(&n, d, training);
  if (rc) return rc;
  if (!bytes) return set_error(SRES_ERR_INVALID_ARG, "rcan: null output");
  *bytes = n.total;
  return SRES_OK;
}

extern "C" int sres_rcan_num_segments(const sres_rcan_desc* d) { return d ? d->n_groups + 2 : -1; }

extern "C" int sres_rcan_segment_params(const sres_rcan_desc* d, int seg, int64_t* offset, int64_t* count) {
  Net n;
  int rc = build_net(&n, d, 0);
  if (rc) return rc;
  if (!offset || !count || seg < 0 || seg > d->n_groups + 1) return set_error(SRES_ERR_INVALID_ARG, "rcan: bad segment");
  if (seg == 0) { *offset = n.bt_w; *count = n.n_params - n.bt_w; }
  else if (seg <= d->n_groups) { *offset = n.body0 + (long long)(d->n_groups - seg) * n.group_sz; *count = n.group_sz; }
  else { *offset = 0; *count = n.body0; }
  return SRES_OK;
}

extern "C" int sres_rcan_pack_weights(const sres_rcan_desc* d, const float* params, void* workspace, int training,
                                      void* stream) {
  Net n;
  int rc = build_net(&n, d, training);
  if (rc) return rc;
  if (!params || !workspace) return set_error(SRES_ERR_INVALID_ARG, "rcan: null pointer");
  return pack_all(n, params, (uint8_t*)workspace, (cudaStream_t)stream);
}

extern "C" int sres_rcan_forward(const sres_rcan_desc* d, const float* params, const float* x_nchw, float* out_nchw,
                                 void* workspace, int training, void* stream) {
  Net n;
  int rc = build_net(&n, d, training);
  if (rc) return rc;
  if (!params || !x_nchw || !out_nchw || !workspace) return set_error(SRES_ERR_INVALID_ARG, "rcan: null pointer");
  return forward(n, params, x_nchw, out_nchw, (uint8_t*)workspace, training, stream);
}

extern "C" int sres_async_create(void** out) {
  if (!out) return set_error(SRES_ERR_INVALID_ARG, "async_create: null output");
  AsyncCtx* a = new AsyncCtx();
  cudaError_t e = cudaStreamCreateWithFlags(&a->side, cudaStreamNonBlocking);
  for (int i = 0; i < AsyncCtx::kEvents && e == cudaSuccess; ++i) {
    e = cudaEventCreateWithFlags(&a->fork[i], cudaEventDisableTiming);
    if (e == cudaSuccess) e = cudaEventCreateWithFlags(&a->done[i], cudaEventDisableTiming);
    a->live[i] = false;
  }
  if (e != cudaSuccess) { delete a; return set_cuda_error(e, "async_create"); }
  *out = a;
  return SRES_OK;
}

extern "C" int sres_async_destroy(void* ctx) {
  AsyncCtx* a = (AsyncCtx*)ctx;
  if (!a) return SRES_OK;
  for (int i = 0; i < AsyncCtx::kEvents; ++i) { cudaEventDestroy(a->fork[i]); cudaEventDestroy(a->done[i]); }
  cudaStreamDestroy(a->side);
  delete a;
  return SRES_OK;
}

extern "C" int sres_rcan_backward(const sres_rcan_desc* d, const float* params, const float* x_nchw,
                                  const float* dout_nchw, float* grads, int accumulate, void* workspace, int seg_begin,
                                  int seg_end, void* async_ctx, void* stream) {
  Net n;
  int rc = build_net(&n, d, 1);
  if (rc) return rc;
  if (!params || !x_nchw || !dout_nchw || !grads || !workspace) return set_error(SRES_ERR_INVALID_ARG, "rcan: null pointer");
  if (seg_begin < 0 || seg_end > d->n_groups + 2 || seg_begin > seg_end)
    return set_error(SRES_ERR_INVALID_ARG, "rcan: bad segment range");
  return backward(n, params, x_nchw, dout_nchw, grads, accumulate, (uint8_t*)workspace, seg_begin, seg_end, (AsyncCtx*)async_ctx,
                  stream);
}

extern "C" int sres_profile_report(char* buf, size_t nbuf) {
  using namespace sres;
  if (!buf || nbuf == 0) return set_error(SRES_ERR_INVALID_ARG, "profile_report: no buffer");
  buf[0] = 0;
  cudaDeviceSynchronize();
  std::lock_guard<std::mutex> lk(g_prof_mu);
  if (!t_prof || t_prof->empty()) return SRES_OK;
  std::map<std::string, std::pair<int, double>> agg;
  double total = 0;
  for (auto& r : *t_prof) {
    float ms = 0;
    cudaEventElapsedTime(&ms, r.a, r.b);
    agg[r.cat].first += 1; agg[r.cat].second += ms; total += ms;
    cudaEventDestroy(r.a); cudaEventDestroy(r.b);
  }
  t_prof->clear();
  size_t off = 0;
  off += snprintf(buf + off, nbuf - off, "total %.3f ms\n", total);
  for (auto& kv : agg)
    if (off < nbuf) off += snprintf(buf + off, nbuf - off, "%-40s n=%5d  %8.3f ms  %5.1f%%  avg %7.1f us\n", kv.first.c_str(),
                                    kv.second.first, kv.second.second, 100.0 * kv.second.second / total,
                                    1e3 * kv.second.second / kv.second.first);
  return SRES_OK;
}
```

Before: 2336.

## Fold channel-attention backward into conv pair epilogues for interior RCAB layers

For interior residual channel-attention blocks, the separate CA-backward pass that materialised dt2 is replaced by a small coefficient kernel. The spatially constant attention-gradient term is folded through the next conv as per-border-class biases, and the gate scaling is applied in the preceding conv-pair epilogue. The conv2 weight gradient contribution from that constant term is recovered analytically from pooled t1 sums and border strips, in new side-stream kernels. This removes a full-tensor read/write pass per block, at the cost of heavier epilogues, new template variants and more complex correctness reasoning.

```diff
diff --git a/include/sres_b200.h b/include/sres_b200.h
--- a/include/sres_b200.h
+++ b/include/sres_b200.h
@@ -65,6 +65,8 @@
 SRES_API size_t sres_conv_pair_flag_bytes(int B, int H, int W);
 SRES_API int sres_conv_pair_supported(const sres_conv_args* first, const sres_conv_args* second);
 SRES_API int sres_conv3x3_pair(const sres_conv_args* first, const sres_conv_args* second, void* flags, void* stream);
+SRES_API int sres_conv3x3_pair_bwd_fold(const sres_conv_args* first, const sres_conv_args* second, void* flags,
+                                        const float* cls_bias, float* t1_part, const float* gate, void* u_bf16, void* stream);
 
 typedef struct sres_rcab_chain_args {
   void* xb_bf16;
@@ -136,6 +138,13 @@
 SRES_API int sres_ca_bwd_apply(const float* grad_f32, const float* tile_part, const float* w1, const float* b1,
                                const float* w2, const float* b2, int hidden, const float* save_mean, void* dt2_bf16,
                                float* save_ds, int B, int H, int W, void* stream);
+SRES_API int sres_ca_bwd_coef(const float* tile_part, const float* w1, const float* b1, const float* w2, const float* b2,
+                              int hidden, const float* conv2_w, const float* save_mean, float* save_ds, float* coef,
+                              float* cls_bias, int B, int H, int W, void* stream);
+SRES_API size_t sres_ca_fold_wgrad_scratch_bytes(int nlayers, int B);
+SRES_API int sres_ca_fold_wgrad(const void* t1_bf16, int64_t t1_stride, const float* t1_part, int64_t part_stride,
+                                const float* coef, int64_t coef_stride, float* conv2_grads, int64_t layer_stride, int nlayers, int B, int H, int W,
+                                void* scratch, size_t scratch_bytes, void* stream);
 SRES_API size_t sres_ca_param_grads_scratch_bytes(int nlayers, int B);
 SRES_API int sres_ca_param_grads(const float* params_first, float* grads_first, int64_t layer_stride, int nlayers,
                                  const float* save_mean, const float* save_ds, int B, int hidden, int accumulate,
diff --git a/super-resolution-climate_b200/csrc/ca.cu b/super-resolution-climate_b200/csrc/ca.cu
--- a/super-resolution-climate_b200/csrc/ca.cu
+++ b/super-resolution-climate_b200/csrc/ca.cu
@@ -307,6 +307,187 @@
   }
 }
 
+constexpr int kCoefSplit = 4;
+__global__ void __launch_bounds__(kCaThreads)
+ca_bwd_coef_kernel(CaGeom g, const float* __restrict__ tile_part, const float* __restrict__ w1, const float* __restrict__ b1,
+                   const float* __restrict__ w2, const float* __restrict__ b2, const float* __restrict__ conv2_w,
+                   const float* __restrict__ save_mean, float* __restrict__ save_ds, float* __restrict__ coef,
+                   float* __restrict__ cls_bias) {
+  __shared__ float sm_m[64], sm_h[kCaMaxHidden], sm_dz[64], sm_dh[kCaMaxHidden], sm_c[64];
+  __shared__ float sm_dsr[4][64];
+  __shared__ float sm_a[9 * 64 / kCoefSplit];
+  CaWeights sw;
+  const int b = blockIdx.x, tid = threadIdx.x, ci0 = blockIdx.y * (64 / kCoefSplit);
+  const int lane = tid & 31, wrp = tid >> 5;
+  ca_stage_weights(sw, w1, b1, w2, b2, g.hid);
+  pdl_wait();
+  pdl_launch_dependents();
+  {
+    const int c = tid & 63, part = tid >> 6;
+    const int t0 = (b * g.RP) / g.tile_rows, t1 = ((b + 1) * g.RP - 1) / g.tile_rows;
+    float a = 0.f;
+#pragma unroll 8
+    for (int t = t0; t <= t1; ++t) {
+      const int seg = (t * g.tile_rows >= b * g.RP) ? 0 : 1;
+      a += tile_part[(((size_t)t * 2 + seg) * 4 + part) * 64 + c];
+    }
+    sm_dsr[part][c] = a;
+  }
+  if (tid < 64) sm_m[tid] = save_mean[b * 64 + tid];
+  __syncthreads();
+  ca_hidden(sw, g.hid, sm_m, sm_h);
+  __syncthreads();
+  if (tid < 64) {
+    const float ds = (sm_dsr[0][tid] + sm_dsr[1][tid]) + (sm_dsr[2][tid] + sm_dsr[3][tid]);
+    if (blockIdx.y == 0) save_ds[b * 64 + tid] = ds;
+    const float sg = ca_gate(sw, g.hid, sm_h, tid);
+    sm_dz[tid] = ds * sg * (1.f - sg);
+  }
+  __syncthreads();
+  for (int j = wrp; j < g.hid; j += kCaThreads / 32) {
+    const float v = warp_sum(fmaf(sw.w2t[j * 64 + lane], sm_dz[lane], sw.w2t[j * 64 + 32 + lane] * sm_dz[lane + 32]));
+    if (lane == 0) sm_dh[j] = sm_h[j] > 0.f ? v : 0.f;
+  }
+  __syncthreads();
+  if (tid < 64) {
+    float a = 0.f;
+    for (int j = 0; j < g.hid; ++j) a = fmaf(sw.w1[j * 64 + tid], sm_dh[j], a);
+    const float c = a / float(g.H * g.W);
+    sm_c[tid] = c;
+    if (blockIdx.y == 0) coef[b * 64 + tid] = c;
+  }
+  __syncthreads();
+  constexpr int kN = 9 * 64 / kCoefSplit;
+  if (tid < kN) {
+    const float* wr = conv2_w + (size_t)ci0 * 9 + tid;
+    float a = 0.f;
+#pragma unroll 16
+    for (int co = 0; co < 64; ++co) a = fmaf(__ldg(wr + (size_t)co * 64 * 9), sm_c[co], a);
+    sm_a[tid] = a;
+  }
+  __syncthreads();
+  if (tid < kN) {
+    const int cls = tid / (64 / kCoefSplit), cl = tid % (64 / kCoefSplit), cy = cls / 3, cx = cls % 3;
+    float k = 0.f;
+#pragma unroll
+    for (int ky = 0; ky < 3; ++ky)
+#pragma unroll
+      for (int kx = 0; kx < 3; ++kx)
+        if (!(cy == 0 && ky == 2) && !(cy == 2 && ky == 0) && !(cx == 0 && kx == 2) && !(cx == 2 && kx == 0))
+          k += sm_a[cl * 9 + ky * 3 + kx];
+    cls_bias[((size_t)b * 9 + cls) * 64 + ci0 + cl] = k;
+  }
+}
+
+struct CaFoldBatch {
+  const uint16_t* t1;
+  long long t1_stride;
+  const float* t1_part;
+  long long part_stride;
+  const float* coef;
+  long long coef_stride;
+  float* S;
+  float* grads;
+  long long layer_stride;
+};
+__global__ void __launch_bounds__(kCaThreads)
+ca_fold_sums_kernel(CaGeom g, CaFoldBatch fb) {
+  __shared__ float sm[kCaThreads / 8][64 + 1];
+  __shared__ float sm_v[9][64];
+  const int b = blockIdx.x, layer = blockIdx.y, tid = threadIdx.x, cg = tid & 7;
+  const uint16_t* t1 = fb.t1 + (size_t)layer * fb.t1_stride + (size_t)b * g.RP * 64;
+  if (tid < 64) {
+    const float* part = fb.t1_part + (size_t)layer * fb.part_stride;
+    const int t0 = (b * g.RP) / 128, t1e = ((b + 1) * g.RP - 1) / 128;
+    float a = 0.f;
+    for (int t = t0; t <= t1e; ++t) {
+      const int seg = (t * 128 >= b * g.RP) ? 0 : 1;
+#pragma unroll
+      for (int part_q = 0; part_q < 4; ++part_q) a += part[(((size_t)t * 2 + seg) * 4 + part_q) * 64 + tid];
+    }
+    sm_v[0][tid] = a;
+    const int y1 = g.H - 1, x1 = g.W - 1;
+    sm_v[5][tid] = bf16_lo(t1[(size_t)0 * 64 + tid]);
+    sm_v[6][tid] = bf16_lo(t1[(size_t)x1 * 64 + tid]);
+    sm_v[7][tid] = bf16_lo(t1[(size_t)(y1 * g.P) * 64 + tid]);
+    sm_v[8][tid] = bf16_lo(t1[(size_t)(y1 * g.P + x1) * 64 + tid]);
+  }
+  for (int strip = 0; strip < 4; ++strip) {
+    const int n = strip < 2 ? g.W : g.H;
+    float a[8] = {0, 0, 0, 0, 0, 0, 0, 0};
+    for (int i = tid >> 3; i < n; i += kCaThreads / 8) {
+      const int pix = strip == 0 ? i : strip == 1 ? (g.H - 1) * g.P + i : strip == 2 ? i * g.P : i * g.P + g.W - 1;
+      const uint4 tv = *reinterpret_cast<const uint4*>(t1 + (size_t)pix * 64 + cg * 8);
+      a[0] += bf16_lo(tv.x); a[1] += bf16_hi(tv.x); a[2] += bf16_lo(tv.y); a[3] += bf16_hi(tv.y);
+      a[4] += bf16_lo(tv.z); a[5] += bf16_hi(tv.z); a[6] += bf16_lo(tv.w); a[7] += bf16_hi(tv.w);
+    }
+    __syncthreads();
+#pragma unroll
+    for (int j = 0; j < 8; ++j) sm[tid >> 3][cg * 8 + j] = a[j];
+    __syncthreads();
+    if (tid < 64) {
+      float s = 0.f;
+      for (int i = 0; i < kCaThreads / 8; ++i) s += sm[i][tid];
+      sm_v[1 + strip][tid] = s;
+    }
+  }
+  __syncthreads();
+  for (int e = tid; e < 9 * 64; e += kCaThreads) {
+    const int tap = e >> 6, ci = e & 63, ky = tap / 3, kx = tap % 3;
+    const int ry = ky == 0 ? 2 : ky == 2 ? 1 : 0;
+    const int rx = kx == 0 ? 4 : kx == 2 ? 3 : 0;
+    float v = sm_v[0][ci];
+    if (ry) v -= sm_v[ry][ci];
+    if (rx) v -= sm_v[rx][ci];
+    if (ry && rx) v += sm_v[5 + (ry == 2 ? 2 : 0) + (rx == 4 ? 1 : 0)][ci];
+    fb.S[(((size_t)layer * g.B + b) * 9 + tap) * 64 + ci] = v;
+  }
+}
+
+constexpr int kFoldCo = 16, kFoldChunk = 32;
+__global__ void __launch_bounds__(kCaThreads)
+ca_fold_grad_kernel(CaGeom g, CaFoldBatch fb) {
+  __shared__ float sm_c[kFoldChunk][kFoldCo];
+  const int layer = blockIdx.x, co0 = blockIdx.y * kFoldCo, tid = threadIdx.x;
+  const float* coef = fb.coef + (size_t)layer * fb.coef_stride;
+  const float* S = fb.S + (size_t)layer * g.B * 9 * 64;
+  float acc[3][kFoldCo];
+#pragma unroll
+  for (int i = 0; i < 3; ++i)
+#pragma unroll
+    for (int k = 0; k < kFoldCo; ++k) acc[i][k] = 0.f;
+  float cb = 0.f;
+  for (int b0 = 0; b0 < g.B; b0 += kFoldChunk) {
+    const int nb = min(kFoldChunk, g.B - b0);
+    __syncthreads();
+    for (int i = tid; i < nb * kFoldCo; i += kCaThreads) sm_c[i / kFoldCo][i % kFoldCo] = coef[(size_t)(b0 + i / kFoldCo) * 64 + co0 + i % kFoldCo];
+    __syncthreads();
+    for (int bb = 0; bb < nb; ++bb) {
+      if (tid < kFoldCo) cb += sm_c[bb][tid];
+#pragma unroll
+      for (int i = 0; i < 3; ++i) {
+        const int e = tid + i * kCaThreads;
+        if (e < 9 * 64) {
+          const float sv = S[((size_t)(b0 + bb) * 9) * 64 + e];
+#pragma unroll
+          for (int k = 0; k < kFoldCo; ++k) acc[i][k] = fmaf(sm_c[bb][k], sv, acc[i][k]);
+        }
+      }
+    }
+  }
+  float* dw = fb.grads + (size_t)layer * fb.layer_stride;
+#pragma unroll
+  for (int i = 0; i < 3; ++i) {
+    const int e = tid + i * kCaThreads;
+    if (e < 9 * 64) {
+      const int tap = e >> 6, ci = e & 63;
+#pragma unroll
+      for (int k = 0; k < kFoldCo; ++k) dw[((size_t)(co0 + k) * 64 + ci) * 9 + tap] += acc[i][k];
+    }
+  }
+  if (tid < kFoldCo) dw[64 * 64 * 9 + co0 + tid] += float(g.H * g.W) * cb;
+}
+
 struct CaParamBatch {
   const float* params;
   float* grads;
@@ -505,6 +686,44 @@
   return SRES_OK;
 }
 
+extern "C" int sres_ca_bwd_coef(const float* tile_part, const float* w1, const float* b1, const float* w2, const float* b2,
+                                int hidden, const float* conv2_w, const float* save_mean, float* save_ds, float* coef,
+                                float* cls_bias, int B, int H, int W, void* stream) {
+  CaGeom g;
+  int rc = ca_geom(&g, B, H, W, hidden);
+  if (rc) return rc;
+  if (g.RP < 128 || H < 2 || W < 2) return set_error(SRES_ERR_UNSUPPORTED, "ca_bwd_coef: needs H, W >= 2 and (H+1)*(W+1) >= 128");
+  if (!tile_part || !w1 || !b1 || !w2 || !b2 || !conv2_w || !save_mean || !save_ds || !coef || !cls_bias)
+    return set_error(SRES_ERR_INVALID_ARG, "ca_bwd_coef: null pointer");
+  cudaError_t e = launch_pdl_if(pdl_level() >= 2, ca_bwd_coef_kernel, dim3(B, kCoefSplit), dim3(kCaThreads), ca_weights_bytes(hidden),
+                                (cudaStream_t)stream, g, tile_part, w1, b1, w2, b2, conv2_w, save_mean, save_ds, coef, cls_bias);
+  if (e != cudaSuccess) return set_cuda_error(e, "ca_bwd_coef: launch");
+  return SRES_OK;
+}
+
+extern "C" size_t sres_ca_fold_wgrad_scratch_bytes(int nlayers, int B) {
+  return (size_t)(nlayers > 0 ? nlayers : 0) * (B > 0 ? B : 0) * 9 * 64 * sizeof(float);
+}
+
+extern "C" int sres_ca_fold_wgrad(const void* t1_bf16, int64_t t1_stride, const float* t1_part, int64_t part_stride,
+                                  const float* coef, int64_t coef_stride, float* conv2_grads, int64_t layer_stride, int nlayers, int B, int H,
+                                  int W, void* scratch, size_t scratch_bytes, void* stream) {
+  CaGeom g;
+  int rc = ca_geom(&g, B, H, W, 1);
+  if (rc) return rc;
+  if (g.RP < 128 || H < 2 || W < 2) return set_error(SRES_ERR_UNSUPPORTED, "ca_fold_wgrad: needs H, W >= 2 and (H+1)*(W+1) >= 128");
+  if (!t1_bf16 || !t1_part || !coef || !conv2_grads || !scratch || nlayers <= 0)
+    return set_error(SRES_ERR_INVALID_ARG, "ca_fold_wgrad: bad argument");
+  if (scratch_bytes < sres_ca_fold_wgrad_scratch_bytes(nlayers, B)) return set_error(SRES_ERR_INVALID_ARG, "ca_fold_wgrad: scratch too small");
+  CaFoldBatch fb{(const uint16_t*)t1_bf16, (long long)t1_stride, t1_part, (long long)part_stride, coef, (long long)coef_stride, (float*)scratch,
+                 conv2_grads, (long long)layer_stride};
+  ca_fold_sums_kernel<<<dim3(B, nlayers), kCaThreads, 0, (cudaStream_t)stream>>>(g, fb);
+  SRES_CHECK_LAUNCH("ca_fold_wgrad: sums launch");
+  ca_fold_grad_kernel<<<dim3(nlayers, 64 / kFoldCo), kCaThreads, 0, (cudaStream_t)stream>>>(g, fb);
+  SRES_CHECK_LAUNCH("ca_fold_wgrad: grad launch");
+  return SRES_OK;
+}
+
 extern "C" size_t sres_ca_param_grads_scratch_bytes(int nlayers, int B) {
   return (size_t)(nlayers > 0 ? nlayers : 0) * (B > 0 ? B : 0) * (64 + 2 * kCaMaxHidden) * sizeof(float);
 }
diff --git a/super-resolution-climate_b200/csrc/conv_pair.cu b/super-resolution-climate_b200/csrc/conv_pair.cu
--- a/super-resolution-climate_b200/csrc/conv_pair.cu
+++ b/super-resolution-climate_b200/csrc/conv_pair.cu
@@ -16,6 +16,10 @@
   const float* bias1;
   const float* bias2;
   float* part2;
+  const float* cls_bias;
+  float* part1;
+  const float* gate2;
+  int B;
   unsigned* ready;
   unsigned* consumed;
   long long* timeline;
@@ -24,6 +28,7 @@
 };
 
 constexpr int kPO16 = 1, kPO32 = 2, kPR32 = 4, kPMsk = 8, kPRelu = 16, kPPool = 32, kPDot = 64;
+constexpr int kPCls = 128, kPGate = 256;
 
 __device__ __forceinline__ unsigned ld_acquire_gpu(const unsigned* p) {
   unsigned v;
@@ -58,7 +63,7 @@
 template <int FL>
 __device__ __forceinline__ void epi_rows(const PairParams& p, EpiWarp& w, const float* s_bias, const CUtensorMap* tmO16,
                                          int tile, uint32_t trow) {
-  constexpr bool f_msk = FL & kPMsk, f_relu = FL & kPRelu;
+  constexpr bool f_msk = FL & kPMsk, f_relu = FL & kPRelu, f_cls = FL & kPCls;
   const int lane = w.lane;
   const int row0 = tile * 128 + w.wq * 32;
   const int q = row0 + lane;
@@ -68,6 +73,12 @@
   const int y = rem / p.P;
   const int x = rem - y * p.P;
   const bool pad = (x == p.W) || (y == p.H) || q >= p.npos;
+  const int seg = (b != (tile * 128) / RP) ? 1 : 0;
+  const float* cls = nullptr;
+  if (f_cls) {
+    const int cy = y == 0 ? 0 : (y == p.H - 1 ? 2 : 1), cx = x == 0 ? 0 : (x == p.W - 1 ? 2 : 1);
+    cls = p.cls_bias + (pad ? 4 : (b * 9 + cy * 3 + cx)) * 64;
+  }
   uint32_t raw[32];
   tmem_ld32(trow, raw);
   tmem_ld_wait();
@@ -87,6 +98,13 @@
       v[4 * j + 2] = __uint_as_float(raw[ch * 16 + 4 * j + 2]) + b4.z;
       v[4 * j + 3] = __uint_as_float(raw[ch * 16 + 4 * j + 3]) + b4.w;
     }
+    if (f_cls) {
+#pragma unroll
+      for (int j = 0; j < 4; ++j) {
+        const float4 k4 = __ldg(reinterpret_cast<const float4*>(cls + c0 + 4 * j));
+        v[4 * j + 0] += k4.x; v[4 * j + 1] += k4.y; v[4 * j + 2] += k4.z; v[4 * j + 3] += k4.w;
+      }
+    }
     if (f_relu) {
 #pragma unroll
       for (int j = 0; j < 16; ++j) v[j] = fmaxf(v[j], 0.f);
@@ -103,6 +121,17 @@
         }
       }
     }
+    if (f_cls) {
+      float t[16];
+#pragma unroll
+      for (int j = 0; j < 2; ++j) {
+        const uint4 mk = *reinterpret_cast<const uint4*>(rmk + (((ch * 2 + j) ^ sw3) << 4));
+        const uint32_t w4[4] = {mk.x, mk.y, mk.z, mk.w};
+#pragma unroll
+        for (int e = 0; e < 4; ++e) { t[8 * j + 2 * e] = bf16_lo(w4[e]); t[8 * j + 2 * e + 1] = bf16_hi(w4[e]); }
+      }
+      pool_partials(t, seg, lane, p.part1 + ((long long)tile * 2 * 4 + w.wq) * 64 + c0);
+    }
     if (pad) {
 #pragma unroll
       for (int j = 0; j < 16; ++j) v[j] = 0.f;
@@ -119,6 +148,7 @@
 template <int FL>
 __device__ __forceinline__ void epi_frag(const PairParams& p, EpiWarp& w, const float (&bias8)[8], int tile, uint32_t trow) {
   constexpr bool f_o16 = FL & kPO16, f_o32 = FL & kPO32, f_r32 = FL & kPR32, f_msk = FL & kPMsk, f_dot = FL & kPDot;
+  constexpr bool f_gate = FL & kPGate;
   constexpr bool use_in = f_msk || f_r32;
   const int lane = w.lane;
   const int fm = lane & 3, frq = lane >> 2;
@@ -138,6 +168,19 @@
   const unsigned padmask = __ballot_sync(0xffffffffu, pad);
   const unsigned seg1 = __ballot_sync(0xffffffffu, seg == 1);
   const bool mixed = seg1 != 0u && seg1 != 0xffffffffu;
+  float sg[2][8];
+  if (f_gate) {
+    const int b0 = (tile * 128) / RP;
+#pragma unroll
+    for (int i = 0; i < 2; ++i) {
+      const float* gp = p.gate2 + min(b0 + i, p.B - 1) * 64 + w.half * 32 + 2 * fm;
+#pragma unroll
+      for (int k = 0; k < 4; ++k) {
+        const float2 g2 = __ldg(reinterpret_cast<const float2*>(gp + 8 * k));
+        sg[i][2 * k] = g2.x; sg[i][2 * k + 1] = g2.y;
+      }
+    }
+  }
   tmem_ld_wait();
   if (use_in) mbar_wait(w.bin, (w.n_in - 1) & 1, 6);
   const int sw3 = (frq >> 1) & 3;
@@ -176,6 +219,7 @@
       else { cs0[2 * k] += c0v; cs0[2 * k + 1] += c1v; }
       if (f_o32) *reinterpret_cast<float2*>(row32 + o32) = make_float2(v0, v1);
       if (f_o16) *reinterpret_cast<uint32_t*>(row16 + o16) = pack_bf16x2(v0, v1);
+      if (f_gate) *reinterpret_cast<uint32_t*>(row16 + o16) = pack_bf16x2(v0 * (rs1 ? sg[1][2 * k] : sg[0][2 * k]), v1 * (rs1 ? sg[1][2 * k + 1] : sg[0][2 * k + 1]));
     }
   }
   const float t0 = frag_colsum(cs0, lane);
@@ -497,7 +541,7 @@
       fence_proxy_async_smem();
       __syncwarp();
       if (lane == 0) {
-        if (FL2 & kPO16) tma_store_2d(&tmO16_2, w.s16, w.half * 32, row0);
+        if (FL2 & (kPO16 | kPGate)) tma_store_2d(&tmO16_2, w.s16, w.half * 32, row0);
         if (FL2 & kPO32) tma_store_2d(&tmO32_2, w.s32, w.half * 32, row0);
         bulk_commit();
       }
@@ -576,8 +620,31 @@
   return ((fwd || bwd) && pair_plan(a1->W, fwd, nullptr, nullptr)) ? 1 : 0;
 }
 
+template <int FL1, int FL2>
+static cudaError_t launch_pair(const cudaLaunchConfig_t& cfg, int dev, const CUtensorMap (&tm)[10], const PairParams& p) {
+  auto k = conv3x3_pair_kernel<FL1, FL2>;
+  static thread_local int attr_dev = -1;
+  if (attr_dev != dev) {
+    cudaError_t e = cudaFuncSetAttribute(k, cudaFuncAttributeMaxDynamicSharedMemorySize, 232448);
+    if (e != cudaSuccess) return e;
+    attr_dev = dev;
+  }
+  count_launch();
+  return cudaLaunchKernelEx(&cfg, k, tm[0], tm[1], tm[2], tm[3], tm[4], tm[5], tm[6], tm[7], tm[8], tm[9], p);
+}
+
 extern "C" int sres_conv3x3_pair(const sres_conv_args* a1, const sres_conv_args* a2, void* flags, void* stream_) {
+  return sres_conv3x3_pair_bwd_fold(a1, a2, flags, nullptr, nullptr, nullptr, nullptr, stream_);
+}
+
+extern "C" int sres_conv3x3_pair_bwd_fold(const sres_conv_args* a1, const sres_conv_args* a2, void* flags, const float* cls_bias,
+                                          float* t1_part, const float* gate, void* u_bf16, void* stream_) {
   if (!sres_conv_pair_supported(a1, a2) || !flags) return set_error(SRES_ERR_UNSUPPORTED, "conv pair: flavours / geometry not fusable");
+  const bool fold1 = cls_bias != nullptr, fold2 = gate != nullptr;
+  if (fold1 != (t1_part != nullptr) || fold2 != (u_bf16 != nullptr))
+    return set_error(SRES_ERR_INVALID_ARG, "conv pair: pass cls_bias with t1_part and gate with u_bf16");
+  if ((fold1 || fold2) && (a1->epi_flags == SRES_EPI_RELU || a1->H < 2 || a1->W < 2))
+    return set_error(SRES_ERR_UNSUPPORTED, "conv pair: the channel-attention fold is a backward flavour for H, W >= 2");
   cudaStream_t stream = (cudaStream_t)stream_;
   const bool fwd = a1->epi_flags == SRES_EPI_RELU;
   PairParams p{};
@@ -585,13 +652,13 @@
   p.npos = (int)((long long)a1->B * p.R * p.P);
   p.n_tiles = (p.npos + 127) / 128;
   p.bias1 = a1->bias; p.bias2 = a2->bias; p.part2 = a2->pool_part;
+  p.cls_bias = cls_bias; p.part1 = t1_part; p.gate2 = gate; p.B = a1->B;
   p.ready = (unsigned*)flags; p.consumed = p.ready + p.n_tiles;
   p.timeline = (long long*)a1->debug_timeline;
   {
     static const int fm = [] { const char* e = getenv("SRES_PAIR_FENCE"); return e ? atoi(e) : 8; }();
     p.fence_mode = fm;
   }
-  const int smem_max = 232448;
   size_t smem = 0;
   if (!pair_plan(a1->W, fwd, &p, &smem)) return set_error(SRES_ERR_UNSUPPORTED, "conv pair: no room for the halo ring");
 
@@ -606,6 +673,7 @@
   if ((rc = make_tmap_rows64(&tmW2, a2->wpack_bf16, 9 * 64, 64))) return rc;
   tmO16_2 = tmO1; tmM2 = tmO1; tmR32_2 = tmO1; tmO32_2 = tmO1;
   if (a2->out_bf16 && (rc = make_tmap_rows64_half(&tmO16_2, a2->out_bf16, (uint64_t)p.npos, 32))) return rc;
+  if (u_bf16 && (rc = make_tmap_rows64_half(&tmO16_2, u_bf16, (uint64_t)p.npos, 32))) return rc;
   if (a2->mask_bf16 && (rc = make_tmap_rows64_half(&tmM2, a2->mask_bf16, (uint64_t)p.npos, 32))) return rc;
   if (a2->resid_f32 && (rc = make_tmap_rows64_f32(&tmR32_2, a2->resid_f32, (uint64_t)p.npos, 32))) return rc;
   if (a2->out_f32 && (rc = make_tmap_rows64_f32(&tmO32_2, a2->out_f32, (uint64_t)p.npos, 32))) return rc;
@@ -622,26 +690,14 @@
   at[0].val.programmaticStreamSerializationAllowed = 1;
   cfg.attrs = at;
   cfg.numAttrs = pdl_enabled() ? 1 : 0;
+  const CUtensorMap tm[10] = {tmA1, tmW1, tmO1, tmM1, tmA2, tmW2, tmO16_2, tmM2, tmR32_2, tmO32_2};
+  constexpr int kB1 = kPMsk | kPO16, kB2 = kPR32 | kPO32 | kPMsk | kPDot;
   cudaError_t e;
-  if (fwd) {
-    auto k = conv3x3_pair_kernel<kPRelu | kPO16, kPPool | kPO16>;
-    static thread_local int attr_dev = -1;
-    if (attr_dev != dev) {
-      if ((e = cudaFuncSetAttribute(k, cudaFuncAttributeMaxDynamicSharedMemorySize, smem_max)) != cudaSuccess) return set_cuda_error(e, "conv pair: smem attribute");
-      attr_dev = dev;
-    }
-    count_launch();
-    e = cudaLaunchKernelEx(&cfg, k, tmA1, tmW1, tmO1, tmM1, tmA2, tmW2, tmO16_2, tmM2, tmR32_2, tmO32_2, p);
-  } else {
-    auto k = conv3x3_pair_kernel<kPMsk | kPO16, kPR32 | kPO32 | kPMsk | kPDot>;
-    static thread_local int attr_dev = -1;
-    if (attr_dev != dev) {
-      if ((e = cudaFuncSetAttribute(k, cudaFuncAttributeMaxDynamicSharedMemorySize, smem_max)) != cudaSuccess) return set_cuda_error(e, "conv pair: smem attribute");
-      attr_dev = dev;
-    }
-    count_launch();
-    e = cudaLaunchKernelEx(&cfg, k, tmA1, tmW1, tmO1, tmM1, tmA2, tmW2, tmO16_2, tmM2, tmR32_2, tmO32_2, p);
-  }
+  if (fwd) e = launch_pair<kPRelu | kPO16, kPPool | kPO16>(cfg, dev, tm, p);
+  else if (fold1 && fold2) e = launch_pair<kB1 | kPCls, kB2 | kPGate>(cfg, dev, tm, p);
+  else if (fold1) e = launch_pair<kB1 | kPCls, kB2>(cfg, dev, tm, p);
+  else if (fold2) e = launch_pair<kB1, kB2 | kPGate>(cfg, dev, tm, p);
+  else e = launch_pair<kB1, kB2>(cfg, dev, tm, p);
   if (e != cudaSuccess) return set_cuda_error(e, "conv pair: launch");
   e = cudaGetLastError();
   if (e != cudaSuccess) return set_cuda_error(e, "conv pair: launch");
diff --git a/super-resolution-climate_b200/csrc/rcan_net.cu b/super-resolution-climate_b200/csrc/rcan_net.cu
--- a/super-resolution-climate_b200/csrc/rcan_net.cu
+++ b/super-resolution-climate_b200/csrc/rcan_net.cu
@@ -93,7 +93,7 @@
   size_t o_hf, o_gf[2], o_xf, o_pool_part, o_pool_sum;
   size_t o_sbias;
   size_t o_pair_flags;
-  size_t o_ga, o_gb32, o_gb16, o_dt2[kRing], o_dt1[kRing], o_ds_part, o_wg_ws, o_sw_ws, o_ca_scr, o_du16[4], o_du32[4], o_dres32, o_dres16;
+  size_t o_ga, o_gb32, o_gb16, o_dt2[kRing], o_dt1[kRing], o_ds_part, o_wg_ws, o_sw_ws, o_ca_scr, o_fold[2], o_cls, o_fold_scr, o_du16[4], o_du32[4], o_dres32, o_dres16;
   size_t total;
   int n_xb, n_t;
   long long cidx(int g, int r, int which) const { return (long long)g * per + 2 * r + which; }
@@ -104,6 +104,9 @@
 };
 
 static size_t align_up(size_t v, size_t a = 1024) { return (v + a - 1) / a * a; }
+
+static size_t fold_part_floats(int B, int H, int W) { return (size_t)sres_conv_mtiles(B, H, W) * 2 * 4 * 64; }
+static size_t fold_layer_bytes(int B, int H, int W) { return (fold_part_floats(B, H, W) + (size_t)B * 64) * 4; }
 
 static int build_net(Net* n, const sres_rcan_desc* d, int training) {
   if (!d) return set_error(SRES_ERR_INVALID_ARG, "rcan: null description");
@@ -194,6 +197,9 @@
       const int bpi = sres_ca_blocks_per_image(d->B, d->H, d->W);
       n->o_ds_part = take((size_t)d->B * (bpi > 0 ? bpi : 1) * 64 * 4);
       n->o_ca_scr = take(sres_ca_param_grads_scratch_bytes(R, d->B));
+      for (int k = 0; k < 2; ++k) n->o_fold[k] = take((size_t)R * fold_layer_bytes(d->B, d->H, d->W));
+      n->o_cls = take((size_t)d->B * 9 * 64 * 4);
+      n->o_fold_scr = take(sres_ca_fold_wgrad_scratch_bytes(R, d->B));
     }
     n->o_wg_ws = take(sres_conv_wgrad_workspace_bytes());
     n->o_sw_ws = take(sres_small_wgrad_workspace_bytes());
@@ -477,7 +483,7 @@
     return rc;
   }
   template <class F>
-  int run_side(F fn) {
+  int run_side(F fn, const void* reads = nullptr) {
     if (!ax || join_per_segment()) return fn(st);
     const int i = ax->next;
     ax->next = (i + 1) % AsyncCtx::kEvents;
@@ -489,6 +495,7 @@
     e = cudaEventRecord(ax->done[i], ax->side);
     if (e != cudaSuccess) return set_cuda_error(e, "backward: side event");
     for (int k = 0; k < SRES_WGRAD_MAX_JOBS; ++k) ax->bufs[i][k] = nullptr;
+    ax->bufs[i][0] = reads;
     ax->live[i] = true;
     return SRES_OK;
   }
@@ -595,6 +602,19 @@
       float* Gg = Gr + n.off_gt(g);
       RC(wq.push(XB(xb0 + R), gb16, B, H, W, Gg, Gg + kConvW, 64, 1, 0, accumulate));
       float* dot_part = (float*)(ws + n.o_pool_part);
+      const bool fold = fused_dot && H >= 2 && W >= 2 && R >= 3 && [&] {
+        const sres_conv_args a1 = conv64_args(gb16, WD(0), nullptr, B, H, W, nullptr, ws + n.o_dt1[0], 0, nullptr, nullptr, nullptr, gb16);
+        const sres_conv_args a2 = conv64_args(ws + n.o_dt1[0], WD(0), nullptr, B, H, W, gb32, nullptr, SRES_EPI_DOT, dot_part, gb32,
+                                              nullptr, gb16);
+        return sres_conv_pair_supported(&a1, &a2) != 0;
+      }();
+      auto folded = [&](int r) { return fold && r >= 1 && r <= R - 2; };
+      uint8_t* fold_reg = ws + n.o_fold[g & 1];
+      const size_t fold_stride = fold_layer_bytes(B, H, W);
+      auto FPART = [&](int r) { return (float*)(fold_reg + (size_t)r * fold_stride); };
+      auto FCOEF = [&](int r) { return FPART(r) + fold_part_floats(B, H, W); };
+      float* cls = (float*)(ws + n.o_cls);
+      if (fold) RC(wq.before_write(fold_reg));
       RC(conv64(gb16, WD(n.cidx_gt(g)), nullptr, B, H, W, st, gb32, nullptr, fused_dot ? SRES_EPI_DOT : 0,
                 fused_dot ? dot_part : nullptr, nullptr, nullptr, fused_dot ? T2(g * R + R - 1) : nullptr));
       for (int r = R - 1; r >= 0; --r) {
@@ -609,18 +629,34 @@
         float* dsv = (float*)(ws + n.o_ds) + (size_t)ti * B * 64;
         void* dt2 = ws + n.o_dt2[ti % ring_len()];
         void* dt1 = ws + n.o_dt1[ti % ring_len()];
-        RC(wq.before_write(dt2));
-        { PROF("ca_bwd");
-        if (fused_dot) RC(sres_ca_bwd_apply(gb32, dot_part, w1, b1, w2, b2, n.hid, mean, dt2, dsv, B, H, W, st));
-        else RC(sres_ca_bwd(gb32, T2(ti), w1, b1, w2, b2, n.hid, mean, (float*)(ws + n.o_ds_part), dt2, dsv, B, H, W, st)); }
+        if (folded(r)) {
+          PROF("ca_bwd_coef");
+          RC(sres_ca_bwd_coef(dot_part, w1, b1, w2, b2, n.hid, pr + kConvW + 64, mean, dsv, FCOEF(r), cls, B, H, W, st));
+        } else {
+          RC(wq.before_write(dt2));
+          PROF("ca_bwd");
+          if (fused_dot) RC(sres_ca_bwd_apply(gb32, dot_part, w1, b1, w2, b2, n.hid, mean, dt2, dsv, B, H, W, st));
+          else RC(sres_ca_bwd(gb32, T2(ti), w1, b1, w2, b2, n.hid, mean, (float*)(ws + n.o_ds_part), dt2, dsv, B, H, W, st));
+        }
         RC(wq.push(T1(ti), dt2, B, H, W, gr + kConvW + 64, gr + 2 * kConvW + 64, 64, 1, 0, accumulate));
         RC(wq.before_write(dt1));
         if (r > 0) {
-          RC(conv64_pair(conv64_args(dt2, WD(n.cidx(g, r, 1)), nullptr, B, H, W, nullptr, dt1, 0, nullptr, nullptr, nullptr, T1(ti)),
-                         conv64_args(dt1, WD(n.cidx(g, r, 0)), nullptr, B, H, W, gb32, nullptr, fused_dot ? SRES_EPI_DOT : 0,
-                                     fused_dot ? dot_part : nullptr, gb32, nullptr, fused_dot ? T2(ti - 1) : nullptr),
-                         ws + n.o_pair_flags + (size_t)(ti & 1) * sres_conv_pair_flag_bytes(B, H, W), st,
-                         "conv pair bwd (dgrad2 -> dgrad1 +rmw +dot)"));
+          const sres_conv_args a1 = conv64_args(dt2, WD(n.cidx(g, r, 1)), nullptr, B, H, W, nullptr, dt1, 0, nullptr, nullptr, nullptr, T1(ti));
+          const sres_conv_args a2 = conv64_args(dt1, WD(n.cidx(g, r, 0)), nullptr, B, H, W, gb32, nullptr, fused_dot ? SRES_EPI_DOT : 0,
+                                                fused_dot ? dot_part : nullptr, gb32, nullptr, fused_dot ? T2(ti - 1) : nullptr);
+          if (folded(r) || folded(r - 1)) {
+            void* u = ws + n.o_dt2[(ti - 1) % ring_len()];
+            if (folded(r - 1)) RC(wq.before_write(u));
+            PROF(folded(r) ? (folded(r - 1) ? "conv pair bwd +ca fold (bias, u)" : "conv pair bwd +ca fold (bias)")
+                           : "conv pair bwd +ca fold (u)");
+            RC(sres_conv3x3_pair_bwd_fold(&a1, &a2, ws + n.o_pair_flags + (size_t)(ti & 1) * sres_conv_pair_flag_bytes(B, H, W),
+                                          folded(r) ? cls : nullptr, folded(r) ? FPART(r) : nullptr,
+                                          folded(r - 1) ? (const float*)(ws + n.o_s) + (size_t)(ti - 1) * B * 64 : nullptr,
+                                          folded(r - 1) ? u : nullptr, st));
+          } else {
+            RC(conv64_pair(a1, a2, ws + n.o_pair_flags + (size_t)(ti & 1) * sres_conv_pair_flag_bytes(B, H, W), st,
+                           "conv pair bwd (dgrad2 -> dgrad1 +rmw +dot)"));
+          }
           RC(wq.push(XB(xb0 + r), dt1, B, H, W, gr, gr + kConvW, 64, 1, 0, accumulate));
         } else {
           RC(conv64(dt2, WD(n.cidx(g, r, 1)), nullptr, B, H, W, st, nullptr, dt1, 0, nullptr, nullptr, nullptr, T1(ti)));
@@ -635,10 +671,14 @@
       PROF("ca_param_grads");
       if (join_per_segment()) RC(wq.join_all());
       RC(wq.run_side([&](void* s) {
+        if (fold)
+          RC(sres_ca_fold_wgrad(T1(g * R + 1), (int64_t)(bf / 2), FPART(1), (int64_t)(fold_stride / 4), FCOEF(1), (int64_t)(fold_stride / 4),
+                                Gr + n.off_rcab(g, 1) + kConvW + 64, n.rcab_sz, R - 2, B, H, W, ws + n.o_fold_scr,
+                                sres_ca_fold_wgrad_scratch_bytes(R, B), s));
         return sres_ca_param_grads(P + first, Gr + first, n.rcab_sz, R, (const float*)(ws + n.o_mean) + (size_t)g * R * B * 64,
                                    (const float*)(ws + n.o_ds) + (size_t)g * R * B * 64, B, n.hid, accumulate,
                                    ws + n.o_ca_scr, sres_ca_param_grads_scratch_bytes(R, B), s);
-      }));
+      }, fold ? fold_reg : nullptr));
     } else if (seg == G + 1) {
       PROF("head wgrad");
       RC(sres_small_in_wgrad(ga, dres32, x, B, d.cin, H, W, Gr + n.head_w, Gr + n.head_b, accumulate, ws + n.o_sw_ws,
```

New measurement: 2168 (median of 6 runs). 0.928x the previous value.
